# ChrisHekmanOtoy/opencl_render

Measured on AMD Instinct MI355X. Metric: Mrays/s (primary rays; each also traces its shadow/bounce rays) at ms/frame = ms_per_step, higher is better.
Workload: dtype f32

## Files before the change

include/raytrace_hip.h:

```cpp
#ifndef RAYTRACE_HIP_H
#define RAYTRACE_HIP_H

#include <stddef.h>
#include <stdint.h>
#include <time.h>

#ifdef __cplusplus
extern "C" {
#endif

#ifndef __OPENCL_CL_H
typedef int32_t  cl_int;
typedef uint32_t cl_uint;
typedef uint16_t cl_ushort;
typedef uint8_t  cl_uchar;
typedef int8_t   cl_char;
typedef float    cl_float;
typedef cl_uint  cl_bool;
typedef union { cl_float s[2]; } __attribute__((aligned(8)))  cl_float2;
typedef union { cl_uint  s[2]; } __attribute__((aligned(8)))  cl_uint2;
typedef union { cl_int   s[2]; } __attribute__((aligned(8)))  cl_int2;
typedef union { cl_float s[4]; } __attribute__((aligned(16))) cl_float4;
typedef union { cl_int   s[4]; } __attribute__((aligned(16))) cl_int4;
typedef union { cl_uchar s[4]; } __attribute__((aligned(4)))  cl_uchar4;
// ... 345 lines not shown
    char name[64];
    cl_float kd[3];
    cl_float ke[3]; cl_int hasKe;
    cl_float dissolve;
    cl_float reflect; cl_int hasReflect;
    char map[5][256];
} rtHipObjMaterial;
typedef struct rtHipObjData {
    cl_uint pointCount; cl_float3 *points;
    cl_uint polygonCount; cl_int *polygons; cl_float3 *cornerNormals; cl_float2 *cornerUv; cl_int *polygonMaterial;
    cl_uint materialCount; rtHipObjMaterial *materials;
} rtHipObjData;
int  rtHipObjRead(const char *path, rtHipObjData *out);
void rtHipObjFree(rtHipObjData *data);

int rtHipImageRead(const char *path, cl_uint *width, cl_uint *height, cl_uchar3 **pixels);

enum { RT_PROJ_SPHERICAL = 0, RT_PROJ_CYLINDRICAL = 1, RT_PROJ_FLAT = 2, RT_PROJ_CUBIC = 3, RT_PROJ_FRONTAL = 4, RT_PROJ_SPATIAL = 5,
       RT_PROJ_UVW = 6, RT_PROJ_SHRINKWRAP = 7, RT_PROJ_VOLUMESHADER = 10 };
int rtHipProjectUv(int projection, const cl_float point[3], const cl_float normal[3], cl_float offsetX, cl_float offsetY, cl_float lengthX,
                   cl_float lengthY, int tile, cl_float uv[2]);

void rtHipPlanesToRgb8(cl_uint width, cl_uint height, const cl_ushort *red, const cl_ushort *green, const cl_ushort *blue,
                       cl_uchar *rgb, int lowByteCompat);

int rtHipWriteBmp(const char *path, cl_uint width, cl_uint height, const cl_ushort *red, const cl_ushort *green, const cl_ushort *blue,
                  int lowByteCompat);

int rtHipWritePpm(const char *path, cl_uint width, cl_uint height, const cl_ushort *red, const cl_ushort *green, const cl_ushort *blue);

int rtHipWritePgm(const char *path, cl_uint width, cl_uint height, const cl_ushort *plane);
int rtHipWritePfm(const char *path, cl_uint width, cl_uint height, const cl_float *plane);
int rtHipWritePfmRgb(const char *path, cl_uint width, cl_uint height, const cl_float *rgb);

enum { RT_KAT_RANDF = 0, RT_KAT_SPHERE, RT_KAT_PMODF, RT_KAT_TRI, RT_KAT_PLINE, RT_KAT_BOX, RT_KAT_BIND, RT_KAT_POW, RT_KAT_QUOTIENT,
       RT_KAT_SPHERE_SPLIT, RT_KAT_ACCUM, RT_KAT_OPS };
int rtHipDeviceKat(int device, int op, cl_uint count, const void *in, cl_uint inStride, void *out, cl_uint outStride, const float *table);

enum { RT_SHADE_KAT_TEXEL = 0, RT_SHADE_KAT_NORMAL = 1 };
int rtHipTestShadeKat(const rtHipScene *scene, int op, cl_uint count, const void *in, void *out);

int rtHipTune(const char *key, double value);

int rtHipTestCachePointers(const void *out[6]);

uint64_t rtHipTestHashBytes(const void *bytes, uint64_t count);

int rtHipScenePathClass(const rtHipSceneDesc *desc);

int rtHipTestPathClass(const rtHipScene *scene);

int rtHipTestRoundLog(const rtHipScene *scene, cl_uint *rays, cl_uint n);

int rtHipTestShadeLog(const rtHipScene *scene, cl_uint *listed, cl_uint n);

enum { RT_BUILD_LOG_CAM_THREAD = 0, RT_BUILD_LOG_CAM_GROUP, RT_BUILD_LOG_CAM_ENTRIES, RT_BUILD_LOG_GRID_THREAD, RT_BUILD_LOG_GRID_GROUP,
       RT_BUILD_LOG_GRID_BATCHES, RT_BUILD_LOG_KEY_CAP_FIRST, RT_BUILD_LOG_KEY_CAP_FINAL, RT_BUILD_LOG_GREW, RT_BUILD_LOG_ATTEMPTS,
       RT_BUILD_LOG_PAIRS, RT_BUILD_LOG_FIELDS };
int rtHipTestBuildLog(uint64_t *out, cl_uint n);

enum { RT_SCENE_VIEW_HEADER = 0, RT_SCENE_VIEW_CAM_START, RT_SCENE_VIEW_CAM_END, RT_SCENE_VIEW_TRI_REC, RT_SCENE_VIEW_TRI_SHADE,
       RT_SCENE_VIEW_GRID_BITS, RT_SCENE_VIEW_BLOCK_SPARSE, RT_SCENE_VIEW_PAIR_REC, RT_SCENE_VIEW_CELL_LUT, RT_SCENE_VIEWS };
int rtHipTestSceneView(const rtHipScene *scene, int what, uint64_t firstElement, uint64_t count, void *out);

int rtHipTestSceneCameraList(const rtHipScene *scene, uint64_t first, uint64_t count, cl_uint *out);
int rtHipTestScenePointers(const rtHipScene *scene, const void *out[6]);
int rtHipTestSceneCameraLog(const rtHipScene *scene, uint64_t out[3]);
int rtHipTestSceneCameraTimes(const rtHipScene *scene, double out[2]);

int rtHipTestSceneGeometryLog(const rtHipScene *scene, uint64_t *out, cl_uint n);
int rtHipTestSceneGeometryTimes(const rtHipScene *scene, double ms[4]);

#ifdef __cplusplus
}
#endif
#endif
```

opencl_render_amd/csrc/rt_api.cpp:

```cpp
#include "rt_host.h"
#include "rt_build_shared.h"

#include <cmath>
#include <cstdarg>
#include <cstdio>
#include <cstdlib>
#include <unordered_map>
#include <chrono>

using namespace rthost;

extern "C" hipError_t rtk_launch_trace(const RtDevScene *scene, int counted, hipStream_t stream);
extern "C" hipError_t rtk_launch_prepare(uint32_t triangleCount, const void *vertex, const void *triIndex, const void *triMaterial,
                                         const void *triUv, const void *triNormal, float *triRec, float *triShade, hipStream_t stream);
extern "C" hipError_t rtk_launch_gather_pairs(uint32_t pairCount, const uint32_t *pairTri, const uint32_t *pairInfo, const float *triRec, float *pairRec, hipStream_t stream);
extern "C" hipError_t rtk_launch_detile(const void *tileBuf, const uint32_t *tileIds, uint32_t tileCount, uint32_t width,
                                        uint32_t height, uint32_t tilesX, void *planeR, void *planeG, void *planeB, int accumulate, hipStream_t stream);

extern "C" hipError_t rtp_validate(uint32_t T, uint32_t V, uint32_t M, const void *triIndex, const int *triMaterial, uint64_t camListSize,
                                   const uint32_t *camList, const uint32_t *gridStart, uint64_t gridListSize, const uint32_t *gridList, uint32_t *err,
                                   hipStream_t stream);
extern "C" hipError_t rtp_camera_ranges(uint32_t W, uint32_t H, uint32_t tilesX, const uint32_t *tileIds, uint32_t tileCount, const uint32_t *camStart,
                                        const uint32_t *camEnd, uint64_t camListSize, uint32_t *outStart, uint32_t *outEnd, uint32_t *err, hipStream_t stream);
extern "C" hipError_t rtp_dense_grid(const uint32_t *gridStart, const uint32_t *gridList, unsigned long long *words, uint32_t *sparse, uint32_t *pairOrder,
                                     uint32_t *pairCount, void *scratch, size_t *scratchBytes, hipStream_t stream);

extern "C" hipError_t rtc_scan_bytes(uint32_t n, size_t *bytes);
extern "C" hipError_t rtc_launch_count(const RtCamMoveArgs *args, hipStream_t stream);
extern "C" hipError_t rtc_launch_fill(const RtCamMoveArgs *args, hipStream_t stream);
extern "C" hipError_t rtw_launch_primary(const RtDevScene *scene, const RtWavefront *wf, hipStream_t stream);
extern "C" hipError_t rtw_launch_primary_passes(const RtDevScene *scene, const RtWavefront *wf, uint32_t *passBuf, hipStream_t stream);
extern "C" hipError_t rtw_launch_surface_passes(const RtDevScene *scene, const RtWavefront *wf, float *surfBuf, hipStream_t stream);
extern "C" hipError_t rtw_launch_logic(const RtDevScene *scene, const RtWavefront *wf, uint32_t round, uint32_t blocks, uint32_t slicesIn, const RtRoundMode *next, hipStream_t stream);
extern "C" hipError_t rtw_launch_answer(const RtDevScene *scene, const RtWavefront *wf, uint32_t round, uint32_t blocks, uint32_t slicesIn, const RtShadeList *list,
                                        uint32_t shadeFollows, hipStream_t stream);
extern "C" hipError_t rtw_launch_shade(const RtDevScene *scene, const RtWavefront *wf, uint32_t round, uint32_t blocks, uint32_t slicesIn, const RtRoundMode *next,
                                       const RtShadeList *list, hipStream_t stream);
extern "C" hipError_t rtw_launch_scatter(const RtWavefront *wf, uint32_t round, uint32_t blocks, const RtRoundMode *mode, hipStream_t stream);
extern "C" hipError_t rtw_launch_trace(const RtDevScene *scene, const RtWavefront *wf, uint32_t round, uint32_t blocks, const RtRoundMode *mode, hipStream_t stream);
extern "C" hipError_t rtw_launch_status(const RtWavefront *wf, uint32_t round, uint32_t *shadeCount, hipStream_t stream);
extern "C" hipError_t rtw_launch_accum(const RtDevScene *scene, const RtWavefront *wf, int first, hipStream_t stream);
extern "C" hipError_t rtw_launch_query(const RtDevScene *scene, const void *rays, const uint32_t *excluded, uint32_t count, void *hits,
                                       uint32_t fastQuotient, hipStream_t stream);
extern "C" hipError_t rtw_launch_ao(const RtDevScene *scene, const RtAoArgs *args, hipStream_t stream);
extern "C" hipError_t rtw_launch_motion_mark(const float *triRec, void *ref, uint32_t triangles, hipStream_t stream);
extern "C" hipError_t rtw_launch_motion(const RtDevScene *scene, const RtMotionArgs *args, hipStream_t stream);
extern "C" hipError_t rtw_launch_ao_finish(const RtDevScene *scene, const uint32_t *counter, uint32_t samplesTimesRays, float *out, uint32_t rowMajor,
                                           hipStream_t stream);
extern "C" hipError_t rtw_launch_bake_raster(const RtDevScene *scene, const RtBakeArgs *args, hipStream_t stream);
extern "C" hipError_t rtw_launch_bake_points(const RtDevScene *scene, const RtBakeArgs *args, hipStream_t stream);
extern "C" hipError_t rtw_launch_bake_ao(const RtDevScene *scene, const RtBakeArgs *args, hipStream_t stream);
extern "C" hipError_t rtw_launch_bake_finish(uint32_t texels, const uint32_t *win, const uint32_t *counter, uint32_t rays, float fill, float *out,
                                             uint32_t *tri, hipStream_t stream);
extern "C" hipError_t rtw_launch_bake_dilate(uint32_t W, uint32_t H, const float *src, float *dst, uint32_t last, hipStream_t stream);

namespace {
thread_local std::string g_error;
}

int rthost::fail(const char *fmt, ...)
{
    char buf[512];
    va_list ap;
    va_start(ap, fmt);
    vsnprintf(buf, sizeof buf, fmt, ap);
    va_end(ap);
    g_error = buf;
    return -1;
}

namespace {

Tuning g_tune;
std::mutex g_tuneMutex;
Tuning tuning() { std::lock_guard<std::mutex> lock(g_tuneMutex); return g_tune; }

// ... 75 lines not shown
    D.camStart = ts; D.camEnd = te;
    HIP_OK(hipStreamSynchronize(sc->stream));
    return 0;
}

int build_geometry(rtHipScene *sc, const rtHipSceneDesc *d)
{
    sc->release_part(PART_GEOMETRY);
    sc->curPart = PART_GEOMETRY;
    RtDevScene &D = sc->dev;
    D.triangleCount = d->triangleCount;
    if (d->triangleCount && (!d->triIndex || !d->triMaterial || !d->triUv || !d->triNormal)) return fail("null triangle array");
    if (d->vertexCount && !d->vertex) return fail("null vertex array");
    void *dv = nullptr, *di = nullptr, *dm = nullptr, *du = nullptr, *dn = nullptr;
    const uint64_t T = d->triangleCount, V = d->vertexCount;
    DevScratch scratch;
    HIP_OK(scratch.get(&dv, V * 16)); HIP_OK(scratch.get(&di, T * 16)); HIP_OK(scratch.get(&dm, T * 4));
    HIP_OK(scratch.get(&du, T * 24)); HIP_OK(scratch.get(&dn, T * 48));
    HIP_OK(sc->stager.copy(dv, d->vertex, V * 16));
    HIP_OK(sc->stager.copy(di, d->triIndex, T * 16));
    HIP_OK(sc->stager.copy(dm, d->triMaterial, T * 4));
    HIP_OK(sc->stager.copy(du, d->triUv, T * 24));
    HIP_OK(sc->stager.copy(dn, d->triNormal, T * 48));
    float *rec = nullptr, *shade = nullptr;
    if (sc->alloc<float>(T * 16, &rec) || sc->alloc<float>(T * 24, &shade)) return -1;
    HIP_OK(rtp_validate(d->triangleCount, d->vertexCount, d->materialCount, di, (const int *)dm, 0, nullptr, nullptr, 0, nullptr, sc->prepErr, sc->stream));
    HIP_OK(hipStreamSynchronize(sc->stream));
    if (sc->check_prep() != 0) return -1;
    HIP_OK(rtk_launch_prepare(d->triangleCount, dv, di, dm, du, dn, rec, shade, sc->stream));
    D.triRec = rec; D.triShade = shade;
    HIP_OK(hipStreamSynchronize(sc->stream));
    return 0;
}

void grid_tables(const float *planes, uint8_t *lut, uint32_t *tame)
{
    for (int w = 0; w < 3; ++w) {
        const float *pw = planes + w * (RT_GRID_DIV + 1);
        const float lo = pw[0], step = (pw[RT_GRID_DIV] - pw[0]) / 256.f;
        int c = 0;
        for (int i = 0; i < 256; ++i) {
            const float x = lo + ((float)i + 0.5f) * step;
            while (c < RT_GRID_DIV - 1 && pw[c + 1] < x) ++c;
            lut[w * 256 + i] = (uint8_t)c;
        }
    }
    *tame = 1u;
    for (int i = 0; i < 3 * (RT_GRID_DIV + 1); ++i) {
        const float m = std::fabs(planes[i]);
        if (!(m == 0.f || (m >= 0x1p-60f && m <= 0x1p39f))) *tame = 0u;
    }
}

int build_grid(rtHipScene *sc, const rtHipSceneDesc *d)
{
    sc->release_part(PART_GRID);
    sc->curPart = PART_GRID;
    RtDevScene &D = sc->dev;
    if (!d->boxMin) return fail("null sceneBoxMin");
    std::vector<float> planes(3 * (RT_GRID_DIV + 1));
    for (int w = 0; w < 3; ++w)
        for (int i = 0; i <= RT_GRID_DIV; ++i) planes[w * (RT_GRID_DIV + 1) + i] = d->boxMin[i].s[w];
    if (sc->upload(planes.data(), planes.size(), &D.boxMin, "boxMin")) return -1;
    std::vector<uint8_t> lut(3 * 256);
    grid_tables(planes.data(), lut.data(), &D.planesTame);
    if (sc->upload(lut.data(), lut.size(), &D.cellLut, "cellLut")) return -1;
    const uint64_t cells = (uint64_t)RT_GRID_DIV * RT_GRID_DIV * RT_GRID_DIV;
    if (!d->gridStart) return fail("null scenePixelTriangleListStart");
    const uint64_t listSize = sc->haveGridListSize ? sc->gridListSizeHint : d->gridStart[cells];
    if (listSize && !d->gridList) return fail("null scenePixelTriangleList");
    if (sc->upload(d->gridStart, cells + 1, &D.gridStart, "gridStart")) return -1;
    if (sc->upload(d->gridList, listSize, &D.gridList, "gridList")) return -1;
    HIP_OK(rtp_validate(D.triangleCount, 0, 0, nullptr, nullptr, 0, nullptr, D.gridStart, listSize, D.gridList, sc->prepErr, sc->stream));
    HIP_OK(hipStreamSynchronize(sc->stream));
    if (sc->check_prep() != 0) return -1;
    const size_t blocks = (size_t)(RT_GRID_DIV / 4) * (RT_GRID_DIV / 4) * (RT_GRID_DIV / 4);
    unsigned long long *words = nullptr;
    uint32_t *sparse = nullptr;
    const size_t sparseWords = (size_t)3 * ((63u << 16 | 63u << 8 | 63u) + 1u);
    if (listSize >= RT_PAIR_LIMIT) return fail("scenePixelTriangleList has 2^28 entries or more: pair indices would not fit the trace kernel's records");
    if (sc->alloc<unsigned long long>(blocks, &words) || sc->alloc<uint32_t>(sparseWords, &sparse)) return -1;
    HIP_OK(hipMemsetAsync(sparse, 0, sparseWords * 4, sc->stream));
    DevScratch scratch;
    uint32_t *pairOrder = nullptr, *pairCount = nullptr;
    void *tmp = nullptr;
    size_t tmpBytes = 0;
    HIP_OK(rtp_dense_grid(nullptr, nullptr, nullptr, nullptr, nullptr, nullptr, nullptr, &tmpBytes, sc->stream));
    HIP_OK(scratch.get((void **)&pairOrder, (size_t)listSize * 4)); HIP_OK(scratch.get((void **)&pairCount, (size_t)listSize * 4));
    HIP_OK(scratch.get(&tmp, tmpBytes));
    HIP_OK(rtp_dense_grid(D.gridStart, D.gridList, words, sparse, pairOrder, pairCount, tmp, &tmpBytes, sc->stream));
    float *pairRec = nullptr;
    if (sc->alloc<float>((uint64_t)listSize * 16, &pairRec)) return -1;
    HIP_OK(rtk_launch_gather_pairs((uint32_t)listSize, pairOrder, pairCount, D.triRec, pairRec, sc->stream));
    D.gridBits = words; D.gridBlockSparse = sparse; D.pairRec = pairRec;
    sc->gridListSize = listSize;
    D.cellCount = 0;
    HIP_OK(hipStreamSynchronize(sc->stream));
    return 0;
}

bool materials_admit_opaque_diffuse(const rtHipSceneDesc *d)
{
    for (uint32_t m = 0; m < d->materialCount; ++m)
        for (int c = 1; c < 5; ++c) {
            const uint32_t w = d->matSize[5 * m + c].s[0], h = d->matSize[5 * m + c].s[1];
            if (w == 0u) continue;
            if (w != 1u || h != 1u) return false;
            if (c == 3) continue;
            const cl_uchar *px = d->textures[d->matStart[5 * m + c]].s;
            if (px[0] | px[1] | px[2]) return false;
        }
    return true;
}
bool lights_admit_opaque_diffuse(const rtHipSceneDesc *d) { return d->lightCount <= 1u; }
void derive_path_class(rtHipScene *sc)
{
    sc->dev.pathClass = (sc->tune.logicClass && sc->classMaterials && sc->classLights) ? RT_PATH_CLASS_OPAQUE_DIFFUSE : RT_PATH_CLASS_GENERAL;
}

int build_materials(rtHipScene *sc, const rtHipSceneDesc *d)
{
    sc->release_part(PART_MATERIALS);
    sc->curPart = PART_MATERIALS;
    RtDevScene &D = sc->dev;
    D.materialCount = d->materialCount;
    D.texelCount = d->texturesSize ? d->texturesSize : 1;
    if (sc->upload((const uint32_t *)d->matSize, (uint64_t)d->materialCount * 10, &D.matSize, "materialImageSize")) return -1;
    if (sc->upload((const int32_t *)d->matStart, (uint64_t)d->materialCount * 5, &D.matStart, "materialImageStart")) return -1;
    if (sc->upload((const uint8_t *)d->textures, (uint64_t)d->texturesSize * 4, &D.textures, "textures")) return -1;
    for (uint32_t m = 0; m < d->materialCount * 5; ++m) {
        const uint64_t w = d->matSize[m].s[0], h = d->matSize[m].s[1];
        if (w && ((int64_t)d->matStart[m] < 0 || (uint64_t)d->matStart[m] + w * h > d->texturesSize))
            return fail("material channel %u: %llux%llu texels at %d exceed the %u-texel atlas", m, (unsigned long long)w, (unsigned long long)h, d->matStart[m], d->texturesSize);
    }
    {
        std::vector<uint32_t> rec((size_t)d->materialCount * 8, 0u);
        for (uint32_t m = 0; m < d->materialCount; ++m)
            for (int c = 0; c < 5; ++c) {
                const uint32_t w = d->matSize[5 * m + c].s[0], h = d->matSize[5 * m + c].s[1];
                uint32_t desc = 0u;
                if (w == 1u && h == 1u) {
                    const cl_uchar *px = d->textures[d->matStart[5 * m + c]].s;
                    desc = 0x80000000u | (uint32_t)px[0] | ((uint32_t)px[1] << 8) | ((uint32_t)px[2] << 16);
                } else if (w) desc = 0x40000000u;
                rec[8 * (size_t)m + c] = desc;
            }
        if (sc->upload(rec.data(), rec.size(), &D.matRec, "matRec")) return -1;
    }
    sc->classMaterials = materials_admit_opaque_diffuse(d);
    derive_path_class(sc);
// ... 102 lines not shown
        Wf.lookAhead = T.lookAhead ? 1u : 0u;
        Wf.deadShadow = T.deadShadow ? 1u : 0u;
        const uint64_t qcap = 2 * cap;
        const uint64_t extraCap = (uint64_t)extraFactor * cap;
        const uint64_t ecap = qcap + extraCap;
        if (ecap > 0xfffffff0ull) return fail("tile set too large for one batch");
        Wf.extraCap = (uint32_t)extraCap;
        Wf.sampleBase = 0; Wf.samplesInBatch = (uint32_t)sb;
        if (sc->alloc<unsigned long long>(cap, &Wf.rng) || sc->alloc<uint4>(cap, &Wf.meta) || sc->alloc<float4>(cap, &Wf.outc) ||
            sc->alloc<float4>(cap * RT_RING * 3, &Wf.ring) || sc->alloc<float4>(cap, &Wf.shP) || sc->alloc<float4>(cap, &Wf.shFace) ||
            sc->alloc<float4>(cap, &Wf.shAtt) || sc->alloc<float4>(multiLight ? cap : 1, &Wf.shN) ||
            sc->alloc<unsigned long long>(multiLight ? cap : 1, &Wf.rngL) || sc->alloc<unsigned long long>(cap, &Wf.laKey) ||
            sc->alloc<uint4>(ecap * 4, &Wf.ent[0]) || sc->alloc<uint4>(ecap * 4, &Wf.ent[1]) || sc->alloc<uint2>(cap, &Wf.pathOf[0]) ||
            sc->alloc<uint2>(cap, &Wf.pathOf[1]) || sc->alloc<unsigned long long>(qcap, &Wf.hitKey[0]) || sc->alloc<unsigned long long>(qcap, &Wf.hitKey[1]) ||
            sc->alloc<uint4>(cap, &Wf.res) || sc->alloc<float4>(gpix * sb, &Wf.sampleOut) ||
            sc->alloc<uint32_t>(ecap, &Wf.sortRank) || sc->alloc<uint16_t>(ecap, &Wf.sortTag) || sc->alloc<uint32_t>(ecap, &Wf.sortedIdx) ||
            sc->alloc<uint32_t>((uint64_t)3 * RT_WF_CTL_WORDS, &Wf.ctl) ||
            sc->alloc<uint4>(cap, &G.shade.list) || sc->alloc<uint32_t>((uint64_t)3 * RT_WF_SHARDS, &G.shade.count))
            return -1;
        HIP_OK(hipMemsetAsync(Wf.ctl, 0, sizeof(uint32_t) * 3 * RT_WF_CTL_WORDS, sc->stream));
        HIP_OK(hipMemsetAsync(G.shade.count, 0, sizeof(uint32_t) * 3 * RT_WF_SHARDS, sc->stream));
        HIP_OK(G.hostLog.make(sizeof(uint4) * RT_WF_ROUND_LOG, hipHostMallocMapped));
        memset(G.hostLog, 0, sizeof(uint4) * RT_WF_ROUND_LOG);
        HIP_OK(hipHostGetDevicePointer((void **)&Wf.roundLog, G.hostLog, 0));
        HIP_OK(G.hostCount.make(sizeof(uint32_t) * RT_WF_SHARDS, hipHostMallocDefault));
        HIP_OK(G.hostStatus.make(sizeof(uint32_t) * RT_WF_STATUS_WORDS, hipHostMallocMapped));
        memset(G.hostStatus, 0, sizeof(uint32_t) * RT_WF_STATUS_WORDS);
        HIP_OK(hipHostGetDevicePointer((void **)&Wf.hostStatus, G.hostStatus, 0));
        Wf.spinLimit = T.spinLimit ? T.spinLimit : 16384u;
        Wf.fastQuotient = T.fastQuotient ? 1u : 0u;
        G.queueBlocks = std::min<uint32_t>(cus * 16, (uint32_t)(qcap / 256));
        G.traceBlocks = (uint32_t)(ecap / 256);
        G.logicBlocks = std::min<uint32_t>(cus * 8, (uint32_t)((cap + 255) / 256));
        G.logicBlocks = std::max<uint32_t>(RT_WF_SHARDS / 4, (G.logicBlocks + RT_WF_SHARDS / 4 - 1) / (RT_WF_SHARDS / 4) * (RT_WF_SHARDS / 4));
    }
    HIP_OK(hipStreamSynchronize(sc->stream));
    sc->blocking = T.blocking != 0;
    return 0;
}

void refresh_views(rtHipScene *sc)
{
    const RtDevScene &D = sc->dev;
    for (auto &G : sc->groups) {
        G.dev = D;
        G.dev.tileIds = D.tileIds + G.slot0;
        G.dev.tileCount = G.slot1 - G.slot0;
        G.dev.camStart = D.camStart + (size_t)G.slot0 * RT_TILE_PIXELS;
        G.dev.camEnd = D.camEnd + (size_t)G.slot0 * RT_TILE_PIXELS;
        G.dev.tileBuf = D.tileBuf + (size_t)G.slot0 * 3 * RT_TILE_PIXELS;
    }
}

constexpr uint64_t GEO_PLANE_BYTES = 3 * (RT_GRID_DIV + 1) * 4, GEO_LUT_BYTES = 3 * 256, GEO_START_BYTES = ((uint64_t)RT_GRID_DIV * RT_GRID_DIV * RT_GRID_DIV + 1) * 4,
                   GEO_BITS_BYTES = (uint64_t)(RT_GRID_DIV / 4) * (RT_GRID_DIV / 4) * (RT_GRID_DIV / 4) * 8,
                   GEO_SPARSE_BYTES = (uint64_t)3 * ((63u << 16 | 63u << 8 | 63u) + 1u) * 4;

int clone_part(rtHipScene *dst, const rtHipScene *src, int part)
{
    dst->release_part(part);
    dst->curPart = part;
    std::vector<std::pair<const char *, char *>> moved;
    std::vector<void *> blocks = src->partAllocs[part];
    std::vector<uint64_t> sizes = src->partSizes[part];
    if (src->geo.live >= 0 && (part == PART_GEOMETRY || part == PART_GRID)) {
        const rtHipScene::GeoMove::Set &L = src->geo.set[src->geo.live];
        const uint64_t T = src->dev.triangleCount ? src->dev.triangleCount : 1, n = src->gridListSize ? src->gridListSize : 1;
        if (part == PART_GEOMETRY) { blocks = { L.triRec, L.triShade }; sizes = { T * 64, T * 96 }; }
        else {
            blocks = { L.boxMin, L.cellLut, L.gridStart, L.gridList, L.gridBits, L.sparse, L.pairRec };
            sizes = { GEO_PLANE_BYTES, GEO_LUT_BYTES, GEO_START_BYTES, n * 4, GEO_BITS_BYTES, GEO_SPARSE_BYTES, n * 64 };
        }
    }
    for (size_t i = 0; i < blocks.size(); ++i) {
        char *p = nullptr;
        const uint64_t n = sizes[i];
        if (dst->alloc<char>(n, &p)) return -1;
        HIP_OK(hipMemcpyPeerAsync(p, dst->device, blocks[i], src->device, n, dst->stream));
        moved.emplace_back((const char *)blocks[i], p);
    }
    auto at = [&](const void *old) -> const void * {
        for (auto &m : moved) if (m.first == (const char *)old) return m.second;
        return nullptr;
    };
    const RtDevScene &S = src->dev;
    RtDevScene &D = dst->dev;
#define RT_MOVE(field) D.field = (decltype(D.field))at(S.field)
    if (part == PART_GEOMETRY) { D.triangleCount = S.triangleCount; RT_MOVE(triRec); RT_MOVE(triShade); }
    if (part == PART_GRID) {
        D.planesTame = S.planesTame; D.cellCount = S.cellCount; dst->gridListSize = src->gridListSize;
        RT_MOVE(boxMin); RT_MOVE(cellLut); RT_MOVE(gridStart); RT_MOVE(gridList); RT_MOVE(gridBits); RT_MOVE(gridBlockSparse); RT_MOVE(pairRec);
    }
    if (part == PART_MATERIALS) {
        D.materialCount = S.materialCount; D.texelCount = S.texelCount; RT_MOVE(matSize); RT_MOVE(matStart); RT_MOVE(textures); RT_MOVE(matRec);
        dst->classMaterials = src->classMaterials;
        derive_path_class(dst);
    }
    if (part == PART_LIGHTS) {
        D.lightCount = S.lightCount;
        dst->classLights = src->classLights;
        derive_path_class(dst);
        RT_MOVE(lightType); RT_MOVE(lightPos); RT_MOVE(lightDir); RT_MOVE(lightCol); RT_MOVE(lightRadius); RT_MOVE(lightHalfAtt); RT_MOVE(lightSpread);
    }
#undef RT_MOVE
    HIP_OK(hipStreamSynchronize(dst->stream));
    return 0;
}

int scene_build(rtHipScene *sc, const rtHipSceneDesc *d, const cl_uint *tileIds, cl_uint tileCount, const rtHipScene *like, const Tuning &tune)
{
    if (!d) return fail("null scene description");
    if (d->width == 0 || d->height == 0) return fail("empty image %ux%u", d->width, d->height);
    if (d->sampleCount == 0) return fail("sampleCount must be >= 1");
    if (d->axesDiv != RT_GRID_DIV) return fail("axesDivCount %d unsupported (the reference builds %d, trianglelist.h:110)", d->axesDiv, RT_GRID_DIV);
    if ((uint64_t)d->width * d->height > 0xffffffffull) return fail("image too large");
    HIP_OK(hipSetDevice(sc->device));
    HIP_OK(sc->stream.make(hipStreamNonBlocking));
    sc->tune = tune;
    sc->pipeline = tune.pipeline == RT_HIP_PIPELINE_MEGAKERNEL ? RT_HIP_PIPELINE_MEGAKERNEL : RT_HIP_PIPELINE_WAVEFRONT;
    if (sc->stager.init(sc->stream, tune) != 0) return -1;
    const bool timing = tune.timing != 0;
    auto tLast = std::chrono::steady_clock::now();
    auto mark = [&](const char *what) {
        if (!timing) return;
        (void)hipStreamSynchronize(sc->stream);
        const auto now = std::chrono::steady_clock::now();
        fprintf(stderr, "libraytrace_hip: scene build: %-28s %8.1f ms\n", what, std::chrono::duration<double, std::milli>(now - tLast).count());
        tLast = now;
    };
    rtHipSceneDesc shadowed;
    std::vector<char> hostCopies[10];
    cl_uint gridEnd[1] = { 0 };
    if (d->arraysOnDevice) {
        shadowed = *d;
        auto fetch = [&](int slot, const void *&field, size_t bytes) -> int {
            if (!field || !bytes) return 0;
            hostCopies[slot].resize(bytes);
            HIP_OK(hipMemcpy(hostCopies[slot].data(), field, bytes, hipMemcpyDeviceToHost));
            field = hostCopies[slot].data();
            return 0;
        };
        const uint64_t cells = (uint64_t)RT_GRID_DIV * RT_GRID_DIV * RT_GRID_DIV;
        if (d->gridStart) { HIP_OK(hipMemcpy(gridEnd, d->gridStart + cells, 4, hipMemcpyDeviceToHost)); sc->gridListSizeHint = gridEnd[0]; sc->haveGridListSize = true; }
        if (fetch(0, (const void *&)shadowed.boxMin, (size_t)(RT_GRID_DIV + 1) * 16) || fetch(1, (const void *&)shadowed.matSize, (size_t)d->materialCount * 40) ||
            fetch(2, (const void *&)shadowed.matStart, (size_t)d->materialCount * 20) || fetch(3, (const void *&)shadowed.textures, (size_t)d->texturesSize * 4) ||
            fetch(4, (const void *&)shadowed.lightType, (size_t)d->lightCount * 4) || fetch(5, (const void *&)shadowed.lightPos, (size_t)d->lightCount * 16) ||
            fetch(6, (const void *&)shadowed.lightDir, (size_t)d->lightCount * 16) || fetch(7, (const void *&)shadowed.lightCol, (size_t)d->lightCount * 16) ||
            fetch(8, (const void *&)shadowed.lightRadius, (size_t)d->lightCount * 4) || fetch(9, (const void *&)shadowed.lightHalfAtt, (size_t)d->lightCount * 4))
            return -1;
        d = &shadowed;
    }
    if (build_fixed(sc, d, tileIds, tileCount) != 0) return -1;
    mark("tiles, outputs, bump tables");
    if (like) {
        for (int part : { PART_GEOMETRY, PART_GRID, PART_MATERIALS, PART_LIGHTS })
            if (clone_part(sc, like, part) != 0) return -1;
        mark("geometry, grid, materials, lights (copied from another instance)");
        if (build_camera(sc, d) != 0) return -1;
        mark("camera lists");
    } else {
        if (build_geometry(sc, d) != 0) return -1;
        mark("geometry");
        if (build_grid(sc, d) != 0) return -1;
        mark("grid + dense view");
        if (build_camera(sc, d) != 0) return -1;
        mark("camera lists");
        if (build_materials(sc, d) != 0) return -1;
        if (build_lights(sc, d) != 0) return -1;
        mark("materials + lights");
    }
    HIP_OK(rtp_validate(sc->dev.triangleCount, 0, 0, nullptr, nullptr, sc->camListSize, sc->dev.camList, nullptr, 0, nullptr, sc->prepErr, sc->stream));
    HIP_OK(hipStreamSynchronize(sc->stream));
    HIP_OK(sc->stager.drain());
    if (sc->check_prep() != 0) return -1;
    if (build_wavefront(sc, d->sampleCount) != 0) return -1;
    refresh_views(sc);
    mark("path state buffers");
    return 0;
}

RtRoundMode mode_for(const Tuning &T, uint32_t round, uint64_t rays, uint32_t slicesBefore)
{
    RtRoundMode m;
    m.ordered = (round <= 1u || rays >= T.appendRays) ? 1u : 0u;
    if (T.orderedFirst == 0u && rays < T.appendRays) m.ordered = 0u;
    m.segLen = rays >= T.segRays[0] ? T.segLen[0] : (rays >= T.segRays[1] ? T.segLen[1] : (rays >= T.segRays[2] ? T.segLen[2] : (rays >= T.segRays[3] ? T.segLen[3] : T.segLen[4])));
    if (m.segLen < 1u) m.segLen = 1u;
    uint32_t small = T.smallSlices;
    if (small < 1u || small > RT_WF_SHARDS || (small & (small - 1u))) small = 16u;
    m.slices = rays >= T.sliceRays ? (uint32_t)RT_WF_SHARDS : small;
    if (m.slices > slicesBefore) m.slices = slicesBefore;
    m.groupRays = (uint32_t)std::min<uint64_t>(64, std::max<uint64_t>(16, ((rays + 1099) / 1100 + 15) / 16 * 16));
    if (T.groupRays >= 1u && T.groupRays <= 128u) m.groupRays = T.groupRays;
    return m;
}

int render_wavefront(rtHipScene *sc, hipStream_t st, bool forceDiscovery)
{
    const Tuning &T = sc->tune;
    auto stage = [&](int which, hipStream_t on, auto &&launch) -> hipError_t {
        if (!sc->stageTiming) return launch();
        if (sc->stageEventsUsed == sc->stageEvents.size()) {
            rtHipScene::StageEvent e{};
            hipError_t er = e.a.make();
            if (er != hipSuccess) return er;
            er = e.b.make();
            if (er != hipSuccess) return er;
            sc->stageEvents.push_back(std::move(e));
        }
        rtHipScene::StageEvent &e = sc->stageEvents[sc->stageEventsUsed++];
        e.stage = which;
        hipError_t er = hipEventRecord(e.a, on);
        if (er != hipSuccess) return er;
        er = launch();
        if (er != hipSuccess) return er;
        return hipEventRecord(e.b, on);
    };
    const bool serial = sc->stageTiming || sc->groups.size() == 1;
    auto streamOf = [&](size_t g) { return (serial || g == 0) ? st : sc->groups[g].stream; };
    if (!serial) {
        HIP_OK(hipEventRecord(sc->forkEvent, st));
        for (size_t g = 1; g < sc->groups.size(); ++g) HIP_OK(hipStreamWaitEvent(sc->groups[g].stream, sc->forkEvent, 0));
    }
    const bool watchedFrame = forceDiscovery || sc->blocking || sc->planRounds == 0;
    bool planned = !watchedFrame;
    uint32_t planRounds = sc->planRounds;
    auto round_mode = [&](rtHipScene::Group &G, uint32_t r) -> RtRoundMode {
        if (G.modes.size() <= r) {
            const uint32_t before = G.modes.empty() ? (uint32_t)RT_WF_SHARDS : G.modes.back().slices;
            uint64_t rays = G.guessRays;
            if (planned) rays = r < RT_WF_ROUND_LOG ? G.plan[r].rays : 0;
            else G.guessRays = std::max<uint64_t>(G.guessRays / 4, 1);
            G.modes.resize(r + 1, mode_for(T, r, rays, before));
        }
        return G.modes[r];
    };
    auto trace_blocks = [&](rtHipScene::Group &G, uint32_t r, const RtRoundMode &m) -> uint32_t {
        const uint64_t worst = m.ordered ? G.traceBlocks : 2ull * G.wf.capacity / m.groupRays + 2ull * m.slices;
        if (!planned || r >= RT_WF_ROUND_LOG) return (uint32_t)std::min<uint64_t>(worst, 0x7fffffffu);
        if (T.planGridTiny) return 1;
        const uint64_t rays = G.plan[r].rays;
        const uint64_t extra = std::min<uint64_t>(G.wf.extraCap, G.plan[r].extraSegLen == m.segLen ? G.plan[r].extra : (m.segLen >= 4096u ? 0 : rays * 11));
        const uint64_t want = m.ordered ? ((rays + extra) * 11 / 10 + 255) / 256 + 8 : (rays * 11 / 10 + m.groupRays - 1) / m.groupRays + 2ull * m.slices + 8;
        return (uint32_t)std::max<uint64_t>(std::min<uint64_t>(want, worst), 1);
    };
    auto shade_blocks = [&](rtHipScene::Group &G, uint32_t r, const RtRoundMode &m) -> uint32_t {
        if (!planned || r >= RT_WF_ROUND_LOG) return G.logicBlocks;
        const uint64_t listed = T.planShadeSkip ? 0 : G.plan[r].shade;
        if (listed == 0) return 0;
        const uint64_t perSlice = (listed * 11 / 10 + m.slices - 1) / m.slices + 8;
        const uint64_t waves = (perSlice + 63) / 64 * m.slices, unit = RT_WF_SHARDS / 4;
        return (uint32_t)std::min<uint64_t>(G.logicBlocks, ((waves + 3) / 4 + unit - 1) / unit * unit);
    };
    uint64_t splitRounds = 0;
    auto issue_round = [&](rtHipScene::Group &G, hipStream_t on) -> int {
        const uint32_t r = G.rounds;
        const RtRoundMode mode = r > 0 ? round_mode(G, r) : RtRoundMode{ 0u, 4096u, 64u, (uint32_t)RT_WF_SHARDS };
        if (r > 0) {
            if (mode.ordered) HIP_OK(stage(4, on, [&] { return rtw_launch_scatter(&G.wf, r, G.queueBlocks, &mode, on); }));
            HIP_OK(stage(2, on, [&] { return rtw_launch_trace(&G.dev, &G.wf, r, trace_blocks(G, r, mode), &mode, on); }));
        }
        const RtRoundMode next = round_mode(G, r + 1);
        if (r > 0 && T.logicSplit && G.wf.lookAhead && G.dev.pathClass == RT_PATH_CLASS_OPAQUE_DIFFUSE) {
            const uint32_t shadeBlocks = shade_blocks(G, r, mode);
            ++splitRounds;
            HIP_OK(stage(1, on, [&] { return rtw_launch_answer(&G.dev, &G.wf, r, G.logicBlocks, mode.slices, &G.shade, shadeBlocks ? 1u : 0u, on); }));
            if (shadeBlocks) HIP_OK(stage(1, on, [&] { return rtw_launch_shade(&G.dev, &G.wf, r, shadeBlocks, mode.slices, &next, &G.shade, on); }));
        } else
            HIP_OK(stage(1, on, [&] { return rtw_launch_logic(&G.dev, &G.wf, r, G.logicBlocks, mode.slices, &next, on); }));
        ++G.rounds;
        return 0;
    };
    auto issue_chunk = [&](rtHipScene::Group &G, hipStream_t on) -> int {
        for (uint32_t k = 0; k < 3 && G.rounds < RT_WF_MAX_ROUNDS; ++k)
            if (issue_round(G, on) != 0) return -1;
        HIP_OK(hipMemcpyAsync(G.hostCount, G.wf.ctl + (G.rounds % 3) * RT_WF_CTL_WORDS + RT_WF_CTL_COUNTS, sizeof(uint32_t) * RT_WF_SHARDS, hipMemcpyDeviceToHost, on));
        return 0;
    };
    auto device_error = [&](rtHipScene::Group &G) -> int {
        if (const uint32_t err = G.hostStatus[RT_WF_STATUS_ERROR]) {
            G.hostStatus[RT_WF_STATUS_ERROR] = 0u;
            return fail("wavefront pipeline: device error 0x%x%s -- the frame is invalid", err,
                        (err & RT_WF_ERR_SPIN) ? " (wf_trace_kernel's walk guard tripped: rays were abandoned)" : "");
        }
        return 0;
    };
    auto launch_surface = [&](rtHipScene::Group &G, hipStream_t on) {
        return rtw_launch_surface_passes(&G.dev, &G.wf, sc->surfBuf + (size_t)G.slot0 * RT_SURF_WORDS * RT_TILE_PIXELS, on);
    };
    uint64_t rounds = 0;
    bool anyPlannedBatch = false;
    const uint32_t sampleCount = sc->dev.sampleCount;
    for (uint32_t base = 0; base < sampleCount; base += sc->samplesPerBatch) {
        for (size_t g = 0; g < sc->groups.size(); ++g) {
            rtHipScene::Group &G = sc->groups[g];
            const hipStream_t on = streamOf(g);
            G.wf.sampleBase = base;
            G.wf.samplesInBatch = std::min<uint32_t>(sc->samplesPerBatch, sampleCount - base);
            G.rounds = 0;
            G.modes.clear();
            G.guessRays = (uint64_t)(G.slot1 - G.slot0) * RT_TILE_PIXELS * G.wf.samplesInBatch;
            if (!G.ctlClean) {
                HIP_OK(hipMemsetAsync(G.wf.ctl, 0, sizeof(uint32_t) * (size_t)3 * RT_WF_CTL_WORDS, on));
                HIP_OK(hipMemsetAsync(G.shade.count, 0, sizeof(uint32_t) * (size_t)3 * RT_WF_SHARDS, on));
            }
            G.ctlClean = false;
            if (!planned) memset(G.hostLog, 0, sizeof(uint4) * RT_WF_ROUND_LOG);
            if (sc->passBuf) {
                uint32_t *pass = sc->passBuf + (size_t)G.slot0 * RT_PASS_WORDS * RT_TILE_PIXELS;
                HIP_OK(stage(0, on, [&] {
                    if (base == 0 && sampleCount > 1) {
                        const hipError_t er = hipMemset2DAsync(pass + RT_PASS_HITS * RT_TILE_PIXELS, (size_t)RT_PASS_WORDS * RT_TILE_PIXELS * 4, 0,
                                                               (size_t)RT_TILE_PIXELS * 4, G.slot1 - G.slot0, on);
// ... 1033 lines not shown
    GEO_MEM(geo_set_fit(sc, target, false, 0, 0, true, &allocated), "the spare set of records and grid arrays");
    GEO_MEM(geo_fit(sc, G.material, T * 4, true, &allocated), "the build scratch");
    if (allocated) GEO_HIP(hipMemsetAsync(G.material, 0xff, (size_t)G.material.size, st));

    const void *dVertex = up->vertex, *dIndex = up->triIndex, *dNormal = up->triNormal;
    if (!up->arraysOnDevice) {
        GEO_MEM(geo_fit(sc, G.vertexBuf, V * 16, false, &allocated), "the vertices");
        GEO_HIP(sc->stager.copy(G.vertexBuf, up->vertex, V * 16));
        dVertex = G.vertexBuf;
        GEO_MEM(geo_fit(sc, G.normalBuf, T * 48, true, &allocated), "the corner normals");
        if (up->triNormal) {
            GEO_HIP(sc->stager.copy(G.normalBuf, up->triNormal, T * 48));
            dNormal = G.normalBuf;
        }
    }
    GEO_MEM(geo_fit(sc, G.index[0], T * 16, true, &allocated) && geo_fit(sc, G.index[1], T * 16, true, &allocated), "the index arrays");
    if (up->triIndex) {
        GEO_HIP(sc->stager.copy(G.index[spareIndex], up->triIndex, T * 16));
        dIndex = G.index[spareIndex];
    } else dIndex = G.index[G.retained];
    GEO_HIP(sc->stager.drain());
    GEO_HIP(hipEventRecord(G.ev[0], st));

    GEO_HIP(rtp_validate((uint32_t)T, (uint32_t)V, 0x7fffffffu, dIndex, G.material, 0, nullptr, nullptr, 0, nullptr, sc->prepErr, st));
    GEO_HIP(hipStreamSynchronize(st));
    if (sc->check_prep() != 0) return -5;

    GEO_HIP(rtg_launch_records((uint32_t)T, dVertex, dIndex, dNormal, sc->dev.triShade, N.triRec, N.triShade, st));
    GEO_HIP(hipEventRecord(G.ev[1], st));

    uint64_t pairs = 0, glog[RT_BUILD_LOG_FIELDS] = {};
    G.space.allocated = 0;
    const uint64_t spaceBefore = G.space.bytes;
    const int grc = rt_grid_core_fill(&G.space, (uint32_t)V, (uint32_t)T, dVertex, dIndex, tune.buildKeyCap, listLimit, st, &pairs, glog);
    sc->bytes += G.space.bytes - spaceBefore;
    allocated = allocated || G.space.allocated;
    if (grc == -3) { fail("%s: the grid holds %llu pairs, more than the limit of %llu", who, (unsigned long long)glog[RT_BUILD_LOG_PAIRS], (unsigned long long)listLimit); return -3; }
    if (grc == -7) { fail("%s: a single triangle's fill outgrew its workgroup queue, or the second fill overflowed", who); return -7; }
    if (grc == -4) { fail("%s: no device memory for the grid build", who); return -4; }
    if (grc) { fail("%s: the grid build failed on the device", who); return -2; }
    if (pairs >= RT_PAIR_LIMIT) { fail("%s: the grid holds 2^28 pairs or more: pair indices would not fit the trace kernel's records", who); return -3; }
    GEO_MEM(geo_set_fit(sc, target, true, pairs * 4, pairs * 64, false, &allocated), "the grid list and pair records");
    GEO_MEM(geo_fit(sc, G.pairOrder, pairs * 4, false, &allocated) && geo_fit(sc, G.pairInfo, pairs * 4, false, &allocated), "the pair order");
    if (rt_grid_core_lists(&G.space, pairs, N.gridStart, N.gridList, st) != 0) { fail("%s: sorting the grid's pairs failed on the device", who); return -2; }
    float bm[4 * (RT_GRID_DIV + 1)];
    GEO_HIP(hipMemcpyAsync(bm, G.space.bm, sizeof bm, hipMemcpyDeviceToHost, st));
    GEO_HIP(hipStreamSynchronize(st));
    float planes[3 * (RT_GRID_DIV + 1)];
    uint8_t lut[3 * 256];
    uint32_t tame = 0;
    for (int w = 0; w < 3; ++w)
        for (int i = 0; i <= RT_GRID_DIV; ++i) planes[w * (RT_GRID_DIV + 1) + i] = bm[4 * i + w];
    grid_tables(planes, lut, &tame);
    GEO_HIP(hipMemcpyAsync(N.boxMin, planes, sizeof planes, hipMemcpyHostToDevice, st));
    GEO_HIP(hipMemcpyAsync(N.cellLut, lut, sizeof lut, hipMemcpyHostToDevice, st));
    GEO_HIP(hipEventRecord(G.ev[2], st));

    size_t denseBytes = 0;
    GEO_HIP(rtp_dense_grid(nullptr, nullptr, nullptr, nullptr, nullptr, nullptr, nullptr, &denseBytes, st));
    GEO_MEM(geo_fit(sc, G.denseTmp, denseBytes, true, &allocated), "the dense view's scratch");
    denseBytes = (size_t)G.denseTmp.size;
    GEO_HIP(hipMemsetAsync(N.sparse, 0, GEO_SPARSE_BYTES, st));
    GEO_HIP(rtp_dense_grid(N.gridStart, N.gridList, N.gridBits, N.sparse, G.pairOrder, G.pairInfo, G.denseTmp, &denseBytes, st));
    GEO_HIP(rtk_launch_gather_pairs((uint32_t)pairs, G.pairOrder, G.pairInfo, N.triRec, N.pairRec, st));
    GEO_HIP(hipEventRecord(G.ev[3], st));

    rtHipCamera cam;
    (void)rtHipSceneGetCamera(sc, &cam);
    int camTarget = 0;
    RtCamMoveCtl ctl{};
    float camMs[2] = { 0.f, 0.f };
    if (const int rc = cam_move_build(sc, &cam, N.triRec, N.triShade, listLimit, who, &camTarget, &ctl, camMs)) return rc;
    GEO_HIP(hipEventRecord(G.ev[4], st));
    GEO_HIP(hipStreamSynchronize(st));
    float ms[4] = {};
    for (int i = 0; i < 4; ++i) GEO_HIP(hipEventElapsedTime(&ms[i], G.ev[i], G.ev[i + 1]));
#undef GEO_HIP
#undef GEO_MEM

    RtDevScene &D = sc->dev;
    D.triRec = N.triRec; D.triShade = N.triShade;
    D.boxMin = N.boxMin; D.cellLut = N.cellLut; D.planesTame = tame;
    D.gridStart = N.gridStart; D.gridList = N.gridList; D.gridBits = N.gridBits; D.gridBlockSparse = N.sparse; D.pairRec = N.pairRec;
    sc->gridListSize = pairs;
    G.live = target;
    if (up->triIndex) G.retained = spareIndex;
    sc->cam.args.triRec = N.triRec; sc->cam.args.triShade = N.triShade;
    cam_move_commit(sc, &cam, camTarget, ctl);
    sc->release_part(PART_GEOMETRY);
    sc->release_part(PART_GRID);
    (void)geo_set_fit(sc, target ^ 1, true, N.gridList.size, N.pairRec.size, true, &allocated);
    allocated = allocated || camMade || camCapBefore[0] != sc->cam.list[0].size || camCapBefore[1] != sc->cam.list[1].size;
    G.log[0] = glog[RT_BUILD_LOG_GRID_THREAD]; G.log[1] = glog[RT_BUILD_LOG_GRID_GROUP]; G.log[2] = glog[RT_BUILD_LOG_ATTEMPTS];
    G.log[3] = pairs; G.log[4] = ctl.total; G.log[5] = allocated ? 1 : 0;
    for (int i = 0; i < 4; ++i) G.ms[i] = ms[i];
    return 0;
}

int rtHipTestSceneGeometryLog(const rtHipScene *sc, uint64_t *out, cl_uint n)
{
    if (!sc || (n && !out)) return fail("rtHipTestSceneGeometryLog: null argument");
    for (cl_uint i = 0; i < n; ++i) out[i] = i < 6 ? sc->geo.log[i] : 0;
    return 6;
}

int rtHipTestSceneGeometryTimes(const rtHipScene *sc, double ms[4])
{
    if (!sc || !ms) return fail("rtHipTestSceneGeometryTimes: null argument");
    for (int i = 0; i < 4; ++i) ms[i] = sc->geo.ms[i];
    return 0;
}

int rtHipKernelTime(rtHipScene *sc, double *avgMs, uint64_t *launches)
{
    if (!sc || !avgMs || !launches) return fail("null argument");
    HIP_OK(hipSetDevice(sc->device));
    double total = 0.0;
    for (size_t i = 0; i < sc->eventsUsed; ++i) {
        HIP_OK(hipEventSynchronize(sc->events[i].second));
        float ms = 0.f;
        HIP_OK(hipEventElapsedTime(&ms, sc->events[i].first, sc->events[i].second));
        total += ms;
    }
    *launches = sc->eventsUsed;
    *avgMs = sc->eventsUsed ? total / (double)sc->eventsUsed : 0.0;
    sc->eventsUsed = 0;
    return 0;
}


static std::atomic<cl_bool> g_tableReady{ CL_FALSE };
static std::atomic<int> g_deviceCount{ 0 };
static char g_deviceName[256][256];
static std::mutex g_tableMutex;

// ... 105 lines not shown
            chunks[i].h = chunks[i].p ? hash_chunk(chunks[i].p, chunks[i].n) : mix64(chunks[i].n + 0x51ull);
    };
    std::vector<std::thread> pool;
    for (unsigned t = 1; t < threads; ++t) pool.emplace_back(work);
    work();
    for (auto &t : pool) t.join();
    for (int g = 0; g < 5; ++g) out[g] = 0x12345678u + g;
    for (const Chunk &c : chunks) out[c.group] = mix64(out[c.group] * 0x100000001b3ull ^ c.h);
}

struct SceneCache {
    std::vector<rtHipScene *> scenes;
    std::vector<std::vector<cl_uint>> tiles;
    int first = 0, count = 0, devices = 0;
    Tuning tune;
    uint32_t width = 0, height = 0, sampleCount = 0;
    uint64_t hash[5] = { 0 };
    bool valid = false;
    Dev<uint16_t> planes, gather;
    Dev<uint32_t> gatherIds;
    uint64_t bytes = 0;
    size_t gatherTiles = 0;
    void clear()
    {
        for (rtHipScene *s : scenes) rtHipSceneDestroy(s);
        scenes.clear(); tiles.clear();
        if (valid || planes || gather || gatherIds) {
            if (devices > 0) (void)hipSetDevice(first % devices);
            planes.drop(bytes); gather.drop(bytes); gatherIds.drop(bytes);
        }
        gatherTiles = 0;
        valid = false;
    }
};
SceneCache &g_cache = *new SceneCache();
std::mutex g_cacheMutex;

}

extern "C" {

int rtHipTune(const char *key, double value)
{
    if (!key) return fail("rtHipTune: null key");
    std::lock_guard<std::mutex> lock(g_tuneMutex);
    Tuning &T = g_tune;
    const std::string k = key;
    if (k == "reset") { T = Tuning(); return 0; }
    struct Key { const char *name; uint32_t *f32; uint64_t *f64 = nullptr; double most = 4294967295.0; } table[] = {
        { "stage_mb", &T.stageMb }, { "extra_factor", &T.extraFactor }, { "groups", &T.groups }, { "lookahead", &T.lookAhead },
        { "seg0", &T.segLen[0] }, { "seg1", &T.segLen[1] }, { "seg2", &T.segLen[2] }, { "seg3", &T.segLen[3] }, { "seg4", &T.segLen[4] },
        { "seg_rays0", &T.segRays[0] }, { "seg_rays1", &T.segRays[1] }, { "seg_rays2", &T.segRays[2] }, { "seg_rays3", &T.segRays[3] },
        { "fast_quotient", &T.fastQuotient }, { "spin_limit", &T.spinLimit }, { "append_rays", &T.appendRays }, { "ordered_first", &T.orderedFirst }, { "slice_rays", &T.sliceRays },
        { "small_slices", &T.smallSlices }, { "group_rays", &T.groupRays }, { "blocking", &T.blocking }, { "plan_rounds", &T.planRounds }, { "plan_grid_tiny", &T.planGridTiny }, { "plan_shade_skip", &T.planShadeSkip },
        { "pipeline", &T.pipeline }, { "timing", &T.timing }, { "virtual_devices", &T.virtualDevices }, { "cache", &T.cache }, { "batch_plan", &T.batchPlan },
        { "logic_class", &T.logicClass }, { "dead_shadow", &T.deadShadow }, { "logic_split", &T.logicSplit }, { "query_rays", &T.queryRays, nullptr, 1u << 26 },
        { "ao_samples", &T.aoSamples, nullptr, 1u << 22 }, { "bake_texels", &T.bakeTexels, nullptr, 1u << 24 },
        { "state_mb", nullptr, &T.stateMb, HUGE_VAL }, { "build_key_cap", nullptr, &T.buildKeyCap, 1e18 }, { "build_list_limit", nullptr, &T.buildListLimit },
    };
    for (const Key &e : table) {
        if (k != e.name) continue;
        const double v = value < 0 ? 0 : std::min(value, e.most);
        if (e.f64) *e.f64 = (uint64_t)v; else *e.f32 = (uint32_t)v;
        return 0;
    }
    return fail("rtHipTune: unknown key '%s'", key);
}

int rtHipTestCachePointers(const void *out[6])
{
    if (!out) return -1;
    std::lock_guard<std::mutex> lock(g_cacheMutex);
    if (!g_cache.valid || g_cache.scenes.empty() || !g_cache.scenes[0]) return -2;
    const RtDevScene &D = g_cache.scenes[0]->dev;
    out[0] = D.triRec; out[1] = D.triShade; out[2] = D.pairRec; out[3] = D.matRec; out[4] = D.textures; out[5] = D.camList;
    return 0;
}

int rtHipTestPathClass(const rtHipScene *scene)
{
    if (!scene) return -1;
    return (int)scene->dev.pathClass;
}

int rt_shade_kat_run(const RtDevScene *scene, int op, uint32_t count, const void *in, void *out);

int rtHipTestShadeKat(const rtHipScene *scene, int op, uint32_t count, const void *in, void *out)
{
    if (!scene || (count && (!in || !out))) return -1;
    const RtDevScene &D = scene->dev;
    for (uint32_t i = 0; i < count; ++i) {
        if (op == RT_SHADE_KAT_TEXEL) {
            const int32_t *item = reinterpret_cast<const int32_t *>(in) + 10 * (size_t)i;
            if (D.texelCount == 0u || item[0] < 0 || (uint32_t)item[0] >= D.materialCount || item[1] < 0 || item[1] >= 5) return -1;
        } else if (op == RT_SHADE_KAT_NORMAL) {
            if (reinterpret_cast<const uint32_t *>(in)[12 * (size_t)i] >= D.triangleCount) return -1;
        } else return -1;
    }
    if (op == RT_SHADE_KAT_NORMAL && count && D.texelCount == 0u && D.materialCount) return -1;
    if (hipSetDevice(scene->device) != hipSuccess || hipStreamSynchronize(scene->stream) != hipSuccess) return -3;
    return rt_shade_kat_run(&D, op, count, in, out);
}

int rtHipTestRoundLog(const rtHipScene *scene, uint32_t *rays, uint32_t n)
{
    if (!scene || (n && !rays)) return -1;
    const uint32_t rounds = (uint32_t)std::min<uint64_t>(scene->roundsLast, RT_WF_ROUND_LOG);
    for (uint32_t r = 0; r < n; ++r) {
        uint64_t sum = 0;
        if (r < rounds)
            for (const auto &G : scene->groups) sum += G.hostLog[r].x;
        rays[r] = (uint32_t)std::min<uint64_t>(sum, 0xffffffffu);
    }
    return (int)scene->roundsLast;
}

int rtHipTestShadeLog(const rtHipScene *scene, uint32_t *listed, uint32_t n)
{
    if (!scene || (n && !listed)) return -1;
    const uint32_t rounds = (uint32_t)std::min<uint64_t>(scene->roundsLast, RT_WF_ROUND_LOG);
    for (uint32_t r = 0; r < n; ++r) {
        uint64_t sum = 0;
        if (r < rounds)
            for (const auto &G : scene->groups) sum += G.hostLog[r].w;
        listed[r] = (uint32_t)std::min<uint64_t>(sum, 0xffffffffu);
    }
    return (int)std::min<uint64_t>(scene->splitRoundsLast, 0x7fffffffu);
}

int rtHipTestSceneView(const rtHipScene *scene, int what, uint64_t firstElement, uint64_t count, void *out)
{
    if (!scene) return fail("rtHipTestSceneView: null scene");
    const RtDevScene &D = scene->dev;
    const uint32_t header[5] = { D.planesTame, D.tileCount, D.tilesX, D.triangleCount, (uint32_t)scene->gridListSize };
    const uint64_t tilePixels = (uint64_t)D.tileCount * RT_TILE_PIXELS, blocks = (uint64_t)(RT_GRID_DIV / 4) * (RT_GRID_DIV / 4) * (RT_GRID_DIV / 4);
    struct View { const void *ptr; uint64_t elements, elementBytes; bool host; } v;
    switch (what) {
    case RT_SCENE_VIEW_HEADER: v = { header, 5, 4, true }; break;
    case RT_SCENE_VIEW_CAM_START: v = { D.camStart, tilePixels, 4, false }; break;
    case RT_SCENE_VIEW_CAM_END: v = { D.camEnd, tilePixels, 4, false }; break;
    case RT_SCENE_VIEW_TRI_REC: v = { D.triRec, D.triangleCount, 64, false }; break;
    case RT_SCENE_VIEW_TRI_SHADE: v = { D.triShade, D.triangleCount, 96, false }; break;
    case RT_SCENE_VIEW_GRID_BITS: v = { D.gridBits, blocks, 8, false }; break;
    case RT_SCENE_VIEW_BLOCK_SPARSE: v = { D.gridBlockSparse, (uint64_t)3 * ((63u << 16 | 63u << 8 | 63u) + 1u), 4, false }; break;
    case RT_SCENE_VIEW_PAIR_REC: v = { D.pairRec, scene->gridListSize, 64, false }; break;
    case RT_SCENE_VIEW_CELL_LUT: v = { D.cellLut, 3 * 256, 1, false }; break;
    default: return fail("rtHipTestSceneView: unknown array %d", what);
    }
    if (v.elements > 0x7fffffffull) return fail("rtHipTestSceneView: array %d has %llu elements", what, (unsigned long long)v.elements);
    if (!out) return (int)v.elements;
    if (firstElement > v.elements || count > v.elements - firstElement)
        return fail("rtHipTestSceneView: elements %llu + %llu reach past the %llu of array %d", (unsigned long long)firstElement,
                    (unsigned long long)count, (unsigned long long)v.elements, what);
    if (!count) return 0;
    if (v.host) { memcpy(out, (const char *)v.ptr + firstElement * v.elementBytes, count * v.elementBytes); return 0; }
    if (!v.ptr) return fail("rtHipTestSceneView: the scene does not hold array %d", what);
    HIP_OK(hipSetDevice(scene->device));
    HIP_OK(hipStreamSynchronize(scene->stream));
    HIP_OK(hipMemcpy(out, (const char *)v.ptr + firstElement * v.elementBytes, count * v.elementBytes, hipMemcpyDeviceToHost));
    return 0;
}

int rtHipScenePathClass(const rtHipSceneDesc *desc)
{
    if (!desc) return fail("rtHipScenePathClass: null scene description");
    if (desc->arraysOnDevice) return fail("rtHipScenePathClass: the description's arrays are device memory");
    if (desc->materialCount && (!desc->matSize || !desc->matStart || !desc->textures)) return fail("rtHipScenePathClass: null material array");
    for (uint32_t i = 0; i < desc->materialCount * 5; ++i)
        if (desc->matSize[i].s[0] == 1u && desc->matSize[i].s[1] == 1u && ((int64_t)desc->matStart[i] < 0 || (uint64_t)desc->matStart[i] >= desc->texturesSize))
            return fail("rtHipScenePathClass: material channel %u starts outside the atlas", i);
    return (materials_admit_opaque_diffuse(desc) && lights_admit_opaque_diffuse(desc)) ? RT_PATH_CLASS_OPAQUE_DIFFUSE : RT_PATH_CLASS_GENERAL;
}

uint64_t rtHipTestHashBytes(const void *bytes, uint64_t count) { return hash_chunk((const unsigned char *)bytes, (size_t)count); }

void rtHipCacheClear(void)
{
    std::lock_guard<std::mutex> lock(g_cacheMutex);
    const std::string keep = g_error;
    g_cache.clear();
    g_error = keep;
}

cl_bool RaytraceAll(cl_uint computationType, cl_uint2 cameraImageDimension, cl_float3 cameraEye, cl_float3 cameraEyeToTopLeftVector,
                    cl_float3 cameraLeftToRightPixelSizeVector, cl_float3 cameraTopToBottomPixelSizeVector, cl_float cameraPixelSizeInv,
                    cl_uint *cameraPixelTriangleListStart, cl_uint *cameraPixelTriangleListEnd, cl_uint *cameraPixelTriangleList,
                    ptrdiff_t cameraPixelTriangleListSize, cl_uint sampleCount, cl_uint vertexCount, cl_float3 *vertex,
                    cl_uint triangleCount, cl_int3 *triangleVertexIndex, cl_int *triangleMaterialId, cl_float2 *triangleUv,
                    cl_float3 *triangleNormal, cl_int axesDivCount, cl_float3 *sceneBoxMin, cl_uint *scenePixelTriangleListStart,
                    cl_uint *scenePixelTriangleList, cl_uint materialCount, cl_uint2 *materialImageSize, cl_int *materialImageStart,
                    cl_uint texturesSize, cl_uchar3 *textures, cl_uint lightCount, cl_int *lightType, cl_float3 *lightPosition,
                    cl_float3 *lightDirection, cl_float3 *lightColour, cl_float *lightRadius, cl_float *lightHalfAttenuationDistance,
                    cl_ushort *outputRed, cl_ushort *outputGreen, cl_ushort *outputBlue)
{
    g_error.clear();
    auto refuse = [&](const char *why) -> cl_bool {
        fprintf(stderr, "libraytrace_hip: %s\n", why);
        return CL_FALSE;
    };
// ... 220 lines not shown
```

opencl_render_amd/csrc/rt_host.h:

```cpp
#pragma once
#include "raytrace_hip.h"
#include "rt_device.h"
#include "rt_camera_move.h"
#include "rt_geometry_move.h"
#include "rt_owned.h"

#include <hip/hip_runtime_api.h>

#include <algorithm>
#include <atomic>
#include <cstring>
#include <mutex>
#include <string>
#include <thread>
#include <vector>

#define RT_SURF_BUF_BITS (RT_HIP_PASS_NORMAL | RT_HIP_PASS_ALBEDO)

namespace rthost {

#define RT_INTERNAL __attribute__((visibility("hidden")))

RT_INTERNAL int fail(const char *fmt, ...);

#define HIP_OK(expr)                                                                                   \
    do {                                                                                               \
        hipError_t e_ = (expr);                                                                        \
        if (e_ != hipSuccess) return rthost::fail("%s failed: %s", #expr, hipGetErrorString(e_));      \
    } while (0)

struct Tuning {
    uint32_t stageMb = 32;
    uint32_t extraFactor = 6;
    uint64_t stateMb = 0;
    uint32_t groups = 1;
    uint32_t lookAhead = 1;
    uint32_t segLen[5] = { 4096u, 384u, 96u, 64u, 16u };
    uint32_t segRays[4] = { 700000u, 300000u, 100000u, 30000u };
    uint32_t fastQuotient = 1;
    uint32_t spinLimit = 16384;
    uint32_t appendRays = 300000;
    uint32_t orderedFirst = 1;
    uint32_t sliceRays = 0;
    uint32_t smallSlices = 16;
    uint32_t groupRays = 0;
    uint32_t blocking = 0;
    uint32_t planRounds = 0;
    uint32_t planGridTiny = 0;
    uint32_t planShadeSkip = 0;
    uint32_t pipeline = RT_HIP_PIPELINE_WAVEFRONT;
    uint32_t timing = 0;
    uint32_t virtualDevices = 0;
    uint32_t cache = 1;
    uint32_t batchPlan = 1;
    uint32_t logicClass = 1;
    uint32_t deadShadow = 1;
    uint32_t logicSplit = 1;
    uint64_t buildKeyCap = 0;
    uint64_t buildListLimit = 0xffffffffull;
    uint32_t queryRays = 1u << 20;
    uint32_t aoSamples = 1u << 20;
    uint32_t bakeTexels = 1u << 20;
};

struct DevScratch {
    std::vector<void *> blocks;
    ~DevScratch() { for (void *p : blocks) (void)hipFree(p); }
    hipError_t get(void **out, size_t bytes)
    {
        const hipError_t e = hipMalloc(out, bytes ? bytes : 1);
        if (e == hipSuccess) blocks.push_back(*out);
        return e;
    }
};

struct Stager {
    hipStream_t stream = nullptr;
    char *buf[2] = { nullptr, nullptr };
    hipEvent_t done[2] = { nullptr, nullptr };
    bool used[2] = { false, false };
    size_t size = 0;
    int next = 0;
    struct Pool {
        std::mutex lock;
        std::vector<std::pair<char *, size_t>> idle;
        char *take(size_t bytes)
        {
            {
                std::lock_guard<std::mutex> g(lock);
                for (size_t i = 0; i < idle.size(); ++i)
                    if (idle[i].second == bytes) { char *p = idle[i].first; idle.erase(idle.begin() + i); return p; }
            }
            char *p = nullptr;
            if (hipHostMalloc((void **)&p, bytes, hipHostMallocPortable) != hipSuccess) { (void)hipGetLastError(); return nullptr; }
            return p;
        }
        void give(char *p, size_t bytes)
        {
            std::lock_guard<std::mutex> g(lock);
            if (idle.size() < 8) idle.emplace_back(p, bytes);
            else (void)hipHostFree(p);
        }
    };
    static Pool &pool() { static Pool *p = new Pool(); return *p; }
    int init(hipStream_t st, const Tuning &T)
    {
        stream = st;
        size = (size_t)std::min<uint32_t>(std::max<uint32_t>(T.stageMb, 1u), 4096u) << 20;
        for (int i = 0; i < 2; ++i) HIP_OK(hipEventCreateWithFlags(&done[i], hipEventDisableTiming));
// ... 20 lines not shown
    {
        if (bytes && on_device(src)) return hipMemcpyAsync(dst, src, bytes, hipMemcpyDeviceToDevice, stream);
        for (size_t off = 0; off < bytes;) {
            const size_t n = std::min(size, bytes - off);
            const int i = next;
            next ^= 1;
            if (used[i]) { const hipError_t e = hipEventSynchronize(done[i]); if (e != hipSuccess) return e; }
            if (!buf[i] && !(buf[i] = pool().take(size))) return hipErrorOutOfMemory;
            fill(buf[i], (const char *)src + off, n);
            hipError_t e = hipMemcpyAsync((char *)dst + off, buf[i], n, hipMemcpyHostToDevice, stream);
            if (e != hipSuccess) return e;
            e = hipEventRecord(done[i], stream);
            if (e != hipSuccess) return e;
            used[i] = true;
            off += n;
        }
        return hipSuccess;
    }
    hipError_t drain()
    {
        for (int i = 0; i < 2; ++i) {
            if (used[i]) { const hipError_t e = hipEventSynchronize(done[i]); if (e != hipSuccess) return e; used[i] = false; }
            if (buf[i]) { pool().give(buf[i], size); buf[i] = nullptr; }
        }
        return hipSuccess;
    }
    void destroy()
    {
        for (int i = 0; i < 2; ++i) {
            if (done[i]) { if (used[i]) (void)hipEventSynchronize(done[i]); (void)hipEventDestroy(done[i]); done[i] = nullptr; }
            if (buf[i]) { pool().give(buf[i], size); buf[i] = nullptr; }
        }
    }
};

}

enum { PART_FIXED = 0, PART_CAMERA, PART_GEOMETRY, PART_GRID, PART_MATERIALS, PART_LIGHTS, PART_WAVEFRONT, PART_COUNT };

struct rtHipScene {
    int device = -1;
    rthost::Stream stream;
    RtDevScene dev{};
    std::vector<void *> partAllocs[PART_COUNT];
    std::vector<uint64_t> partSizes[PART_COUNT];
    uint64_t partBytes[PART_COUNT] = { 0 };
    int curPart = PART_FIXED;
    rthost::Stager stager;
    uint32_t *prepErr = nullptr;
    uint64_t camListSize = 0;
    uint64_t gridListSize = 0;
    uint32_t gridListSizeHint = 0;
    bool haveGridListSize = false;
    bool wfMultiLight = false;
    bool classMaterials = false, classLights = false;
    uint64_t bytes = 0;
    std::vector<cl_uint> tileIds;
    uint32_t width = 0, height = 0, tilesX = 0;
    std::vector<std::pair<rthost::Event, rthost::Event>> events;
    size_t eventsUsed = 0;
    int pipeline = RT_HIP_PIPELINE_WAVEFRONT;
    struct Group {
        RtDevScene dev{};
        RtWavefront wf{};
        RtShadeList shade{};
        rthost::Stream stream;
        rthost::Event done;
        uint32_t logicBlocks = 1, traceBlocks = 1, queueBlocks = 1;
        rthost::Pinned<uint32_t> hostCount;
        rthost::Pinned<uint32_t> hostStatus;
        bool ctlClean = false;
        uint32_t rounds = 0;
        uint32_t slot0 = 0, slot1 = 0;
        uint32_t roundsNeeded = 0;
        struct RoundPlan { uint32_t rays = 0, extra = 0, extraSegLen = 0, shade = 0; };
        rthost::Pinned<uint4> hostLog;
        RoundPlan plan[RT_WF_ROUND_LOG], planNext[RT_WF_ROUND_LOG];
        std::vector<RtRoundMode> modes;
        uint64_t guessRays = 0;
    };
    std::vector<Group> groups;
    rthost::Event forkEvent;
    uint32_t samplesPerBatch = 1;
    uint32_t planRounds = 0;
    uint64_t splitRoundsLast = 0;
    bool blocking = false;
    rthost::Tuning tune;
    bool unverified = false;
    hipStream_t lastStream = nullptr;
    rtHipSampleWindow window{}, lastWindow{};
    std::atomic<float> *progress = nullptr;
    float progressBase = 0.f, progressSpan = 0.f;
    struct StageEvent { int stage; rthost::Event a, b; };
    std::vector<StageEvent> stageEvents;
    size_t stageEventsUsed = 0;
    bool stageTiming = false;
    uint64_t roundsLast = 0;
    uint32_t passMask = 0;
    rthost::Dev<uint32_t> passBuf;
    rthost::Dev<float> surfBuf;
    uint32_t queryRays = 0;
    rthost::Dev<> queryDev;
    char *queryHost = nullptr;
    rthost::Dev<> denoiseBuf;
    rthost::Event denoiseEv[4];
    float denoiseMs[3] = {};
    rthost::Dev<> aoBuf;
    uint32_t aoChunk = 0;
    rthost::Event aoDone;
    rthost::Dev<> bakeBuf;
    uint64_t bakeTexels = 0;
    uint32_t bakeChunk = 0;
    rthost::Event bakeDone;
    struct Motion {
        bool have = false;
        rtHipCamera cam{};
        uint32_t triangles = 0;
        rthost::Dev<float4> ref;
        rthost::Dev<> stage;
        rthost::Event marked, done;
    } motion;
    struct Temporal {
        rthost::Dev<> buf, momentsBuf;
        int cur = 0;
        bool valid = false, momentsValid = false;
        rthost::Event ev[5];
        float ms[4] = {};
    } temporal;
    struct CamMove {
        rthost::Dev<> scratch;
        rthost::Dev<uint32_t> start[2], end[2], list[2];
        int live = -1;
        RtCamMoveArgs args{};
        rthost::Event ev[4];
        uint64_t log[3] = {};
        double ms[2] = {};
    } cam;
    struct GeoMove {
        struct Set {
            rthost::Dev<float> triRec, triShade, boxMin, pairRec;
            rthost::Dev<uint8_t> cellLut;
            rthost::Dev<uint32_t> gridStart, gridList, sparse;
            rthost::Dev<unsigned long long> gridBits;
        } set[2];
        int live = -1;
        RtGridSpace space{};
        rthost::Dev<> vertexBuf, normalBuf, index[2], denseTmp;
        rthost::Dev<int> material;
        rthost::Dev<uint32_t> pairOrder, pairInfo;
        int retained = -1;
// ... 90 lines not shown
```

opencl_render_amd/csrc/rt_scene_prep.hip:

```cpp
#include <hip/hip_runtime.h>
#include <hipcub/hipcub.hpp>

#include "rt_device.h"

namespace {

constexpr uint32_t BLOCKS = (RT_GRID_DIV / 4) * (RT_GRID_DIV / 4) * (RT_GRID_DIV / 4);

__global__ __launch_bounds__(256) void rtp_check_triangles(uint32_t T, uint32_t V, uint32_t M, const int4 *__restrict__ triIndex,
                                                           const int *__restrict__ triMaterial, uint32_t *err)
{
    const uint32_t t = blockIdx.x * 256 + threadIdx.x;
    if (t >= T) return;
    const int4 vi = triIndex[t];
    uint32_t bad = 0;
    if ((uint32_t)vi.x >= V || (uint32_t)vi.y >= V || (uint32_t)vi.z >= V) bad |= RT_PREP_ERR_TRI_INDEX;
    if (triMaterial[t] >= (int)M) bad |= RT_PREP_ERR_TRI_MATERIAL;
    if (bad) atomicOr(err, bad);
}

__global__ __launch_bounds__(256) void rtp_check_list(uint64_t n, const uint32_t *__restrict__ list, uint32_t T, uint32_t bit, uint32_t *err)
{
    const uint64_t i = (uint64_t)blockIdx.x * 256 + threadIdx.x;
    if (i < n && list[i] >= T) atomicOr(err, bit);
}

__global__ __launch_bounds__(256) void rtp_check_grid_start(const uint32_t *__restrict__ gridStart, uint32_t *err)
{
    const uint32_t c = blockIdx.x * 256 + threadIdx.x;
    if (gridStart[c] > gridStart[c + 1]) atomicOr(err, RT_PREP_ERR_GRID_MONOTONE);
}

__global__ __launch_bounds__(256) void rtp_camera_tile_major(uint32_t W, uint32_t H, uint32_t tilesX, const uint32_t *__restrict__ tileIds, uint32_t tileCount,
                                                             const uint32_t *__restrict__ camStart, const uint32_t *__restrict__ camEnd, uint64_t camListSize,
                                                             uint32_t *__restrict__ outStart, uint32_t *__restrict__ outEnd, uint32_t *err)
{
    const uint32_t i = blockIdx.x * 256 + threadIdx.x;
    if (i >= tileCount * RT_TILE_PIXELS) return;
    const uint32_t slot = i / RT_TILE_PIXELS, in = i % RT_TILE_PIXELS;
    const uint32_t tile = tileIds[slot];
    const uint32_t gx = (tile % tilesX) * RT_TILE + in % RT_TILE, gy = (tile / tilesX) * RT_TILE + in / RT_TILE;
    uint32_t a = 0, b = 0;
    if (gx < W && gy < H) {
        const uint64_t p = (uint64_t)gy * W + gx;
        a = camStart[p]; b = camEnd[p];
        if (b < a) b = a;
        if ((uint64_t)b > camListSize) { atomicOr(err, RT_PREP_ERR_CAM_RANGE); a = b = 0; }
    }
    outStart[i] = a; outEnd[i] = b;
}

__global__ __launch_bounds__(256) void rtp_block_words(const uint32_t *__restrict__ gridStart, unsigned long long *__restrict__ words,
                                                       uint32_t *__restrict__ blockCells, uint32_t *__restrict__ blockRest)
{
    const uint32_t b = blockIdx.x * 256 + threadIdx.x;
    const uint32_t bx = b & 63u, by = (b >> 6) & 63u, bz = b >> 12;
    unsigned long long w = 0;
    uint32_t cells = 0, rest = 0;
    for (uint32_t z = 0; z < 4; ++z)
        for (uint32_t y = 0; y < 4; ++y) {
            const uint32_t row = (bx * 4) + RT_GRID_DIV * (by * 4 + y) + RT_GRID_DIV * RT_GRID_DIV * (bz * 4 + z);
            uint32_t s[5];
#pragma unroll
            for (int x = 0; x < 5; ++x) s[x] = gridStart[row + x];
#pragma unroll
            for (uint32_t x = 0; x < 4; ++x) {
                const uint32_t n = s[x + 1] - s[x];
                if (n) { w |= 1ull << (x | (y << 2) | (z << 4)); ++cells; rest += n - 1; }
            }
        }
    words[b] = w; blockCells[b] = cells; blockRest[b] = rest;
}

__global__ __launch_bounds__(256) void rtp_block_emit(const uint32_t *__restrict__ gridStart, const uint32_t *__restrict__ gridList,
                                                      const unsigned long long *__restrict__ words, const uint32_t *__restrict__ rank,
                                                      const uint32_t *__restrict__ restBase, const uint32_t *__restrict__ blockCells,
                                                      uint32_t *__restrict__ sparse, uint32_t *__restrict__ pairOrder, uint32_t *__restrict__ pairCount)
{
    const uint32_t b = blockIdx.x * 256 + threadIdx.x;
    const uint32_t bx = b & 63u, by = (b >> 6) & 63u, bz = b >> 12;
    unsigned long long w = words[b];
    const uint32_t first = rank[b];
    const size_t at = (size_t)(bx | (by << 8) | (bz << 16)) * 3;
    sparse[at + 0] = (uint32_t)w; sparse[at + 1] = (uint32_t)(w >> 32); sparse[at + 2] = first;
    const uint32_t cellTotal = rank[BLOCKS - 1] + blockCells[BLOCKS - 1];
    uint32_t dense = first, restAt = cellTotal + restBase[b];
    while (w) {
        const int bit = __ffsll((long long)w) - 1;
        w &= w - 1;
        const uint32_t cell = (bx * 4 + (bit & 3)) + RT_GRID_DIV * (by * 4 + ((bit >> 2) & 3)) + RT_GRID_DIV * RT_GRID_DIV * (bz * 4 + (bit >> 4));
        const uint32_t s = gridStart[cell], n = gridStart[cell + 1] - s;
        pairOrder[dense] = gridList[s];
        pairCount[dense] = (n < RT_PAIR_MANY ? n : RT_PAIR_MANY) | (restAt << 4);
        for (uint32_t i = 1; i < n; ++i) { pairOrder[restAt] = gridList[s + i]; pairCount[restAt] = (i == 1u) ? n : 0u; ++restAt; }
        ++dense;
    }
}

}

extern "C" hipError_t rtp_validate(uint32_t T, uint32_t V, uint32_t M, const void *triIndex, const int *triMaterial, uint64_t camListSize,
                                   const uint32_t *camList, const uint32_t *gridStart, uint64_t gridListSize, const uint32_t *gridList, uint32_t *err,
                                   hipStream_t stream)
{
    if (T && triIndex) hipLaunchKernelGGL(rtp_check_triangles, dim3((T + 255) / 256), dim3(256), 0, stream, T, V, M, (const int4 *)triIndex, triMaterial, err);
    if (camListSize) hipLaunchKernelGGL(rtp_check_list, dim3((uint32_t)((camListSize + 255) / 256)), dim3(256), 0, stream, camListSize, camList, T, RT_PREP_ERR_CAM_ENTRY, err);
    if (gridListSize) hipLaunchKernelGGL(rtp_check_list, dim3((uint32_t)((gridListSize + 255) / 256)), dim3(256), 0, stream, gridListSize, gridList, T, RT_PREP_ERR_GRID_ENTRY, err);
    if (gridStart) hipLaunchKernelGGL(rtp_check_grid_start, dim3((RT_GRID_DIV * RT_GRID_DIV * RT_GRID_DIV) / 256), dim3(256), 0, stream, gridStart, err);
    return hipGetLastError();
}

extern "C" hipError_t rtp_camera_ranges(uint32_t W, uint32_t H, uint32_t tilesX, const uint32_t *tileIds, uint32_t tileCount, const uint32_t *camStart,
                                        const uint32_t *camEnd, uint64_t camListSize, uint32_t *outStart, uint32_t *outEnd, uint32_t *err, hipStream_t stream)
{
    const uint32_t n = tileCount * RT_TILE_PIXELS;
    if (n) hipLaunchKernelGGL(rtp_camera_tile_major, dim3((n + 255) / 256), dim3(256), 0, stream, W, H, tilesX, tileIds, tileCount, camStart, camEnd,
                              camListSize, outStart, outEnd, err);
    return hipGetLastError();
}

extern "C" hipError_t rtp_dense_grid(const uint32_t *gridStart, const uint32_t *gridList, unsigned long long *words, uint32_t *sparse, uint32_t *pairOrder,
                                     uint32_t *pairCount, void *scratch, size_t *scratchBytes, hipStream_t stream)
{
    size_t scanBytes = 0;
    hipError_t e = hipcub::DeviceScan::ExclusiveSum(nullptr, scanBytes, (const uint32_t *)nullptr, (uint32_t *)nullptr, (int)BLOCKS, stream);
    if (e != hipSuccess) return e;
    const size_t need = (size_t)4 * BLOCKS * sizeof(uint32_t) + scanBytes;
    if (!scratch) { *scratchBytes = need; return hipSuccess; }
    if (*scratchBytes < need) return hipErrorInvalidValue;
    uint32_t *blockCells = (uint32_t *)scratch, *blockRest = blockCells + BLOCKS, *rank = blockRest + BLOCKS, *restBase = rank + BLOCKS;
    void *scanTmp = restBase + BLOCKS;
    hipLaunchKernelGGL(rtp_block_words, dim3(BLOCKS / 256), dim3(256), 0, stream, gridStart, words, blockCells, blockRest);
    e = hipcub::DeviceScan::ExclusiveSum(scanTmp, scanBytes, blockCells, rank, (int)BLOCKS, stream);
    if (e != hipSuccess) return e;
    e = hipcub::DeviceScan::ExclusiveSum(scanTmp, scanBytes, blockRest, restBase, (int)BLOCKS, stream);
    if (e != hipSuccess) return e;
    hipLaunchKernelGGL(rtp_block_emit, dim3(BLOCKS / 256), dim3(256), 0, stream, gridStart, gridList, words, rank, restBase, blockCells, sparse, pairOrder,
                       pairCount);
    return hipGetLastError();
}
```

opencl_render_amd/csrc/rt_wavefront.hip:

```cpp
#include "rt_devfuncs.h"

namespace {

enum { WS_RAY = 0, WS_SHADOW = 1 };

__device__ __forceinline__ float4 pack4(V3 v, float w) { return make_float4(v.x, v.y, v.z, w); }
__device__ __forceinline__ V3 xyz(float4 v) { return mk(v.x, v.y, v.z); }

__device__ __forceinline__ void store_single_sample(const RtDevScene &S, uint32_t localPixel, V3 c)
{
    const uint32_t slot = localPixel / RT_TILE_PIXELS, inTile = localPixel % RT_TILE_PIXELS;
    uint16_t *planes = S.tileBuf + (size_t)slot * 3 * RT_TILE_PIXELS + inTile;
    uint32_t samples = S.sampleDivisor;
    asm volatile("" : "+s"(samples));
    const float scale = (float)(0xFFFF) / (float)samples;
    planes[0] = (uint16_t)sat_add_u16(0, c.x, scale);
    planes[RT_TILE_PIXELS] = (uint16_t)sat_add_u16(0, c.y, scale);
    planes[2 * RT_TILE_PIXELS] = (uint16_t)sat_add_u16(0, c.z, scale);
}

__device__ __forceinline__ uint32_t wave_append(uint32_t *counter, bool want)
{
    const unsigned long long mask = __ballot(want);
    if (mask == 0) return 0;
    const uint32_t lane = __lane_id();
    const int leader = __ffsll((long long)mask) - 1;
    uint32_t base = 0;
    if ((int)lane == leader) base = atomicAdd(counter, (uint32_t)__popcll(mask));
    base = __shfl(base, leader, 64);
    return base + (uint32_t)__popcll(mask & ((1ull << lane) - 1ull));
}

__device__ __forceinline__ void wave_append2(uint32_t *counterA, bool wantA, uint32_t *counterB, bool wantB, uint32_t &posA, uint32_t &posB)
{
    const unsigned long long maskA = __ballot(wantA), maskB = __ballot(wantB);
    const uint32_t lane = __lane_id();
    uint32_t base = 0;
    const uint32_t n = (lane == 0u) ? (uint32_t)__popcll(maskA) : (uint32_t)__popcll(maskB);
    if (lane < 2u && n != 0u) base = atomicAdd(lane == 0u ? counterA : counterB, n);
    const unsigned long long below = (1ull << lane) - 1ull;
    posA = (uint32_t)__shfl((int)base, 0, 64) + (uint32_t)__popcll(maskA & below);
    posB = (uint32_t)__shfl((int)base, 1, 64) + (uint32_t)__popcll(maskB & below);
}

__device__ __forceinline__ bool tri_rec_test_flat(const float4 r0, const float4 r1, const float4 r2, const float4 r3, V3 o, V3 d, float tmin,
                                                  float tmax, float &t, float &l1, float &l2)
{
    const V3 a = mk(r0.x, r0.y, r0.z), ab = mk(r0.w, r1.x, r1.y), ac = mk(r1.z, r1.w, r2.x), n = mk(r2.y, r2.z, r2.w);
    const V3 ao = sub3(o, a);
    t = -dot3(n, ao) / dot3(n, d);
    const V3 ap = sub3(along(o, t, d), a);
    const float ap_ab = dot3(ap, ab);
    const float ap_ac = dot3(ap, ac);
// ... 205 lines not shown
}

#ifndef RT_WF_MAXSEG
#define RT_WF_MAXSEG 12
#endif
struct DdaState { uint32_t cell; float dx, dy, dz; };

__device__ __forceinline__ uint32_t axis_state_at(const float *planes, uint32_t c0, float oa, float da, float tau, float &head,
                                                  const uint8_t *lut = nullptr, float lutScale = 0.f)
{
    const bool pos = (0.f <= da);
    const int limit = pos ? (int)(RT_GRID_DIV - 1 - c0) : (int)c0;
    const float p = oa + tau * da;
    int g = 0;
    bool search = true;
    if (lut) {
        const int i = min(255, max(0, (int)((p - planes[0]) * lutScale)));
        const int a = lut[max(i - 1, 0)], b = lut[min(i + 1, 255)];
        g = lut[i];
        search = b - a > 4;
    }
    if (search) {
        g = 0;
#pragma unroll
        for (int div = RT_GRID_DIV / 2; div >= 1; div /= 2)
            if (planes[g + div] < p) g += div;
    }
    int m = pos ? g - (int)c0 : (int)c0 - g;
    m = m < 0 ? 0 : (m > limit ? limit : m);
    while (m >= 1 && !((planes[pos ? (int)c0 + m : (int)c0 - m + 1] - oa) / da <= tau)) --m;
    float next = (planes[pos ? (int)c0 + m + 1 : (int)c0 - m] - oa) / da;
    while (m < limit && next <= tau) {
        ++m;
        next = (planes[pos ? (int)c0 + m + 1 : (int)c0 - m] - oa) / da;
    }
    head = next;
    return pos ? c0 + (uint32_t)m : c0 - (uint32_t)m;
}

__device__ __forceinline__ uint32_t cell_of(const float *planes, V3 p)
{
    int cx = 0, cy = 0, cz = 0;
#pragma unroll
    for (int div = RT_GRID_DIV / 2; div >= 1; div /= 2) {
        if (planes[cx + div] < p.x) cx += div;
        if (planes[(RT_GRID_DIV + 1) + cy + div] < p.y) cy += div;
        if (planes[2 * (RT_GRID_DIV + 1) + cz + div] < p.z) cz += div;
    }
    return (uint32_t)cx | ((uint32_t)cy << 8) | ((uint32_t)cz << 16);
}

struct EntryPlan { DdaState start; uint32_t endCell, visits; float te; };

__device__ __forceinline__ EntryPlan plan_ray(const float *planes, V3 o, V3 d, float tmin, float tmax, bool haveStart = false, uint32_t startCell = 0u,
                                              const uint8_t *lut = nullptr, const float *lutScale = nullptr)
{
    EntryPlan p;
    const V3 lo = mk(planes[0], planes[RT_GRID_DIV + 1], planes[2 * (RT_GRID_DIV + 1)]);
    const V3 hi = mk(planes[RT_GRID_DIV], planes[2 * RT_GRID_DIV + 1], planes[3 * RT_GRID_DIV + 2]);
    V3 from = along(o, tmin, d);
    bind_in_cube(from, d, lo, hi);
    p.start.cell = startCell;
    if (!haveStart) p.start.cell = cell_of(planes, from);
    p.te = RT_INF;
    V3 to;
    if (tmax < RT_INF) {
        to = along(o, tmax, d);
        bind_in_cube(to, d, lo, hi);
    } else {
        if (d.x != 0.f) { const float t = (((0.f <= d.x) ? hi.x : lo.x) - o.x) / d.x; if (t < p.te) p.te = t; }
        if (d.y != 0.f) { const float t = (((0.f <= d.y) ? hi.y : lo.y) - o.y) / d.y; if (t < p.te) p.te = t; }
        if (d.z != 0.f) { const float t = (((0.f <= d.z) ? hi.z : lo.z) - o.z) / d.z; if (t < p.te) p.te = t; }
        to = (p.te < RT_INF) ? along(o, p.te, d) : from;
    }
    uint32_t last;
    if (lut && !(tmax < RT_INF)) {
        const float fx = (to.x - lo.x) * lutScale[0], fy = (to.y - lo.y) * lutScale[1], fz = (to.z - lo.z) * lutScale[2];
        const int ix = min(255, max(0, (int)fx)), iy = min(255, max(0, (int)fy)), iz = min(255, max(0, (int)fz));
        last = (uint32_t)lut[ix] | ((uint32_t)lut[256 + iy] << 8) | ((uint32_t)lut[512 + iz] << 16);
    } else last = cell_of(planes, to);
    p.endCell = (tmax < RT_INF) ? last : 0xffffffffu;
    const int cx = (int)(p.start.cell & 255u), cy = (int)((p.start.cell >> 8) & 255u), cz = (int)(p.start.cell >> 16);
    p.start.dx = (planes[cx + ((0 <= d.x) ? 1 : 0)] - o.x) / d.x;
    p.start.dy = (planes[(RT_GRID_DIV + 1) + cy + ((0 <= d.y) ? 1 : 0)] - o.y) / d.y;
    p.start.dz = (planes[2 * (RT_GRID_DIV + 1) + cz + ((0 <= d.z) ? 1 : 0)] - o.z) / d.z;
    p.visits = (uint32_t)(abs((int)(last & 255u) - cx) + abs((int)((last >> 8) & 255u) - cy) + abs((int)(last >> 16) - cz)) + 1u;
    return p;
}

__device__ __forceinline__ uint32_t segments_of(const EntryPlan &p, V3 d, float tmax, uint32_t segLen)
{
    const float ta = fminf(p.start.dx, fminf(p.start.dy, p.start.dz));
    const bool plain = !(tmax < RT_INF) && d.x != 0.f && d.y != 0.f && d.z != 0.f && p.te < RT_INF && -RT_INF < ta && ta < p.te &&
                       p.start.dx == p.start.dx && p.start.dy == p.start.dy && p.start.dz == p.start.dz && p.start.dx < RT_INF &&
                       p.start.dy < RT_INF && p.start.dz < RT_INF;
    if (!plain || p.visits <= segLen + segLen / 4) return 1u;
    const uint32_t n = (p.visits + segLen - 1) / segLen;
    return n > RT_WF_MAXSEG ? (uint32_t)RT_WF_MAXSEG : n;
}

__device__ __forceinline__ bool cut_at(float ta, float te, uint32_t k, uint32_t n, float &tau)
{
    tau = ta + (te - ta) * ((float)k / (float)n);
    return ta <= tau && tau < te;
}

#ifndef RT_WF_LOGIC_WAVES
#define RT_WF_LOGIC_WAVES 3
#endif
#ifndef RT_WF_LOGIC_WAVES_FIRST
#define RT_WF_LOGIC_WAVES_FIRST 3
#endif
#ifndef RT_WF_LOGIC_WAVES_FIRST_ORDERED
#define RT_WF_LOGIC_WAVES_FIRST_ORDERED 3
#endif
#ifndef RT_WF_LOGIC_WAVES_LEAN_FIRST
#define RT_WF_LOGIC_WAVES_LEAN_FIRST 4
#endif
#ifndef RT_WF_LOGIC_WAVES_LEAN
#define RT_WF_LOGIC_WAVES_LEAN 4
#endif
#define RT_WF_LIGHTS_LDS 64
#ifdef RT_DIAG_LOGIC
#define DG(i) dg[i] = diag_stamp()
#else
#define DG(i)
#endif
__device__ __forceinline__ void class_light_accum(V3 &face, float ndl, bool front, float lmax, float4 lc, V3 atten)
{
    const float mag = __builtin_fabsf(ndl);
    const float x = lmax / lc.w;
    const float e = mag * half_falloff(x);
    if ((0.f <= ndl) == front) {
        face.x += (1.f - face.x) * atten.x * e * lc.x;
        face.y += (1.f - face.y) * atten.y * e * lc.y;
        face.z += (1.f - face.z) * atten.z * e * lc.z;
    }
}
__device__ __forceinline__ void class_shade_end(V3 &out, V3 P, V3 face)
{
    out.x += P.x * face.x;
    out.y += P.y * face.y;
    out.z += P.z * face.z;
}

__device__ __forceinline__ void log_round_rays(const RtWavefront &W, const uint32_t *ctlIn, uint32_t round, uint32_t lane, uint32_t wave)
{
    __shared__ uint32_t sumWave[4], maxWave[4];
// ... 229 lines not shown
        const uint32_t at = blockIdx.x * 256 + threadIdx.x;
        active = at < total;
        if (active) mine = W.sortedIdx[at];
        for (int i = threadIdx.x; i < 3 * (RT_GRID_DIV + 1); i += 256) planes[i] = S.boxMin[i];
        __syncthreads();
    } else {
        const uint32_t group = min(mode.groupRays, (uint32_t)RT_WF_GROUP_RAYS);
        __shared__ uint32_t pieceWave[4], pieceAt[2];
        uint32_t sl = 0, row = 0, count = 0;
        {
            static_assert(2 * RT_WF_SHARDS == 512, "two queue slices per thread");
            const uint32_t s0 = threadIdx.x, s1 = 256u + threadIdx.x;
            const uint32_t c0 = s0 < 2u * mode.slices ? slice_count(ctl, mode.slices, s0) : 0u, c1 = s1 < 2u * mode.slices ? slice_count(ctl, mode.slices, s1) : 0u;
            const uint32_t p0 = (c0 + group - 1u) / group, p1 = (c1 + group - 1u) / group;
            uint32_t i0 = p0, i1 = p1;
#pragma unroll
            for (int off = 1; off < 64; off <<= 1) {
                const uint32_t u0 = __shfl_up(i0, off, 64), u1 = __shfl_up(i1, off, 64);
                if ((int)lane >= off) { i0 += u0; i1 += u1; }
            }
            if (lane == 63) { pieceWave[wave] = i0; }
            __syncthreads();
            uint32_t before0 = 0, all0 = 0;
            for (uint32_t w = 0; w < 4; ++w) { if (w < wave) before0 += pieceWave[w]; all0 += pieceWave[w]; }
            __syncthreads();
            if (lane == 63) { pieceWave[wave] = i1; }
            __syncthreads();
            uint32_t before1 = all0, all1 = all0;
            for (uint32_t w = 0; w < 4; ++w) { if (w < wave) before1 += pieceWave[w]; all1 += pieceWave[w]; }
            const uint32_t first0 = before0 + i0 - p0, first1 = before1 + i1 - p1;
            if (blockIdx.x == 0 && threadIdx.x == 0 && all1 > gridDim.x) atomicOr(W.hostStatus + RT_WF_STATUS_ERROR, RT_WF_ERR_GRID);
            if (blockIdx.x >= all1) return;
            if (first0 <= blockIdx.x && blockIdx.x < first0 + p0) { pieceAt[0] = s0; pieceAt[1] = blockIdx.x - first0; }
            if (first1 <= blockIdx.x && blockIdx.x < first1 + p1) { pieceAt[0] = s1; pieceAt[1] = blockIdx.x - first1; }
            __syncthreads();
            sl = pieceAt[0]; row = pieceAt[1];
            count = slice_count(ctl, mode.slices, sl);
        }
        for (int i = threadIdx.x; i < 3 * (RT_GRID_DIV + 1); i += 256) planes[i] = S.boxMin[i];
        __syncthreads();
        const uint32_t rowsUsed = (count + group - 1u) / group;
        __shared__ uint32_t planWave[2];
        uint32_t n = 0;
        const uint32_t local = row + threadIdx.x * rowsUsed;
        const bool planner = threadIdx.x < group && local < count;
        if (planner) {
            const uint32_t q = slice_first(W, mode.slices, sl) + local;
            const uint4 *e = W.ent[par] + 4 * (size_t)q;
            const uint32_t excl = reinterpret_cast<const uint32_t *>(e)[3];
            const float tmin = __uint_as_float(reinterpret_cast<const uint32_t *>(e)[7]);
            const uint4 c2 = e[2], c3 = e[3];
            const V3 o = mk(__uint_as_float(c2.x), __uint_as_float(c2.y), __uint_as_float(c2.z)), d = mk(__uint_as_float(c3.x), __uint_as_float(c3.y), __uint_as_float(c3.z));
            const float tmax = __uint_as_float(c2.w);
            const EntryPlan plan = plan_ray(planes, o, d, tmin, tmax);
            n = segments_of(plan, d, tmax, mode.segLen);
            rayO[threadIdx.x] = pack4(o, tmin); rayD[threadIdx.x] = pack4(d, tmax);
            rayX[threadIdx.x] = make_uint4(excl, q, plan.start.cell, plan.endCell);
            rayT[threadIdx.x] = make_float4(plan.start.dx, plan.start.dy, plan.start.dz, plan.te);
        }
        if (wave < 2) {
            uint32_t sum = n;
#pragma unroll
            for (int off = 32; off >= 1; off >>= 1) sum += __shfl_xor(sum, off, 64);
            if (lane == 0) planWave[wave] = sum;
        }
        __syncthreads();
        const uint32_t all = planWave[0] + planWave[1];
        __syncthreads();
        if (wave < 2) {
            const uint32_t raysHere = min(group, (count - row + rowsUsed - 1u) / rowsUsed);
            if (all > 256u && n > 1u) n = max(1u, n * (256u - raysHere) / all);
            uint32_t incl = n;
#pragma unroll
            for (int off = 1; off < 64; off <<= 1) {
                const uint32_t up = __shfl_up(incl, off, 64);
                if ((int)lane >= off) incl += up;
            }
            if (lane == 63) planWave[wave] = incl;
            n = incl - n;
        }
        __syncthreads();
        if (wave < 2) {
            const uint32_t nextFirst = (uint32_t)__shfl_down((int)n, 1, 64);
            const uint32_t first = n + (wave == 1 ? planWave[0] : 0u), mineN = (lane == 63 ? planWave[wave] : nextFirst) - n;
            segFirst[threadIdx.x] = first;
            if (threadIdx.x == 127) segFirst[128] = planWave[0] + planWave[1];
            for (uint32_t k = 0; k < mineN; ++k) segOwner[first + k] = (uint8_t)threadIdx.x;
        }
        __syncthreads();
        segments = segFirst[128];
    }

    for (uint32_t pass = 0; pass < 1u; ++pass) {
    uint32_t q = 0, excluded = RT_NONE, cell = 0, endCell = 0xffffffffu, seg = 0;
    V3 o = mk(0, 0, 0), d = mk(1, 1, 1);
    float tmin = 0.f, tmax = 0.f, dx = 0.f, dy = 0.f, dz = 0.f;
    if (ORDERED) {
        if (active) {
            const uint4 *e = W.ent[par] + 4 * (size_t)mine;
            const uint4 c0 = e[0], c1 = e[1], c2 = e[2], c3 = e[3];
            q = c0.x; cell = c0.y & 0xffffffu; endCell = c0.z; excluded = c0.w;
            dx = __uint_as_float(c1.x); dy = __uint_as_float(c1.y); dz = __uint_as_float(c1.z); tmin = __uint_as_float(c1.w);
            o = mk(__uint_as_float(c2.x), __uint_as_float(c2.y), __uint_as_float(c2.z)); tmax = __uint_as_float(c2.w);
            d = mk(__uint_as_float(c3.x), __uint_as_float(c3.y), __uint_as_float(c3.z));
            seg = c3.w >> 24;
        }
    } else {
// ... 961 lines not shown
```

opencl_render_amd/csrc/rt_wf_logic_body.h:

```cpp
    __shared__ Shared sh;
    __shared__ float4 ltPosRadius[RT_WF_LIGHTS_LDS], ltDirSpread[RT_WF_LIGHTS_LDS], ltColHalf[RT_WF_LIGHTS_LDS];
    __shared__ int ltType[RT_WF_LIGHTS_LDS];
    __shared__ uint32_t waveHist[ORDERED ? 4 : 1][RT_WF_SORT_BINS], waveBase[ORDERED ? 4 : 1][RT_WF_SORT_BINS];
    __shared__ uint8_t cellLut[ORDERED ? 3 * 256 : 4];
    __shared__ uint8_t itemOwner[ORDERED ? 4 : 1][2 * 64 * (RT_WF_MAXSEG - 1)];
    __shared__ uint32_t itemWord[ORDERED ? 4 : 1][ORDERED ? 2 * 64 * (RT_WF_MAXSEG - 1) : 1];
    __shared__ float lutScale[3];
    static_assert(RT_WF_SORT_BINS == 64, "one class per lane");
    sh.unit255[threadIdx.x] = (float)threadIdx.x / 255.f;
    if (ORDERED) {
        float *pl = &sh.planes[0][0];
        for (int i = threadIdx.x; i < 3 * (RT_GRID_DIV + 1); i += 256) pl[i] = S.boxMin[i];
        waveHist[threadIdx.x >> 6][threadIdx.x & 63] = 0u;
        if (threadIdx.x < 3 * 256 / 4) reinterpret_cast<uint32_t *>(cellLut)[threadIdx.x] = reinterpret_cast<const uint32_t *>(S.cellLut)[threadIdx.x];
        if (threadIdx.x < 3) lutScale[threadIdx.x] = 256.f / (S.boxMin[threadIdx.x * (RT_GRID_DIV + 1) + RT_GRID_DIV] - S.boxMin[threadIdx.x * (RT_GRID_DIV + 1)]);
    }
    if (threadIdx.x < RT_WF_LIGHTS_LDS && threadIdx.x < S.lightCount) {
        const uint32_t k = threadIdx.x;
        ltType[k] = S.lightType[k];
        ltPosRadius[k] = make_float4(S.lightPos[4 * k], S.lightPos[4 * k + 1], S.lightPos[4 * k + 2], S.lightRadius[k]);
        ltDirSpread[k] = make_float4(S.lightDir[4 * k], S.lightDir[4 * k + 1], S.lightDir[4 * k + 2], S.lightSpread[k]);
        ltColHalf[k] = make_float4(S.lightCol[4 * k], S.lightCol[4 * k + 1], S.lightCol[4 * k + 2], S.lightHalfAtt[k]);
    }
    __syncthreads();
// ... 572 lines not shown
                    W.shFace[a] = pack4(face, front ? 1.f : 0.f);
                    if (attStored) W.shAtt[a] = pack4(atten, 0.f);
                    if (multiLight) {
                        W.rngL[a] = rngL;
                        if (shadedNow) W.shN[a] = pack4(n, 0.f);
                    }
                }
            }
        }
        uint32_t slot, slotLa;
        wave_append2(&ctlOut[RT_WF_CTL_COUNTS + outShard], emit, &ctlOut[RT_WF_CTL_COUNTS + RT_WF_SHARDS + outShard], emitLa, slot, slotLa);
        slot += outShard * sliceCapOut;
        slotLa += W.capacity + outShard * sliceCapOut;
        asm volatile("" : "+v"(a), "+v"(slot), "+v"(slotLa));
        if (slot != 0xfffffff0u) DG(8);
        const uint32_t copy = waveId % RT_WF_SORT_COPIES;
        if (!ORDERED) {
#pragma unroll 1
            for (int which = 0; which < 2; ++which) {
                const bool has = which ? emitLa : emit;
                if (!has) continue;
                const V3 o = which ? lo3 : ro, d = which ? ld3v : rd;
                const float tmin = which ? latmin : rtmin, tmax = which ? RT_INF : rtmax;
                const uint32_t excluded = which ? laexcl : rexcl, mine = which ? slotLa : slot;
                uint4 *e = W.ent[outq] + 4 * (size_t)mine;
                if (!which) W.pathOf[outq][mine] = make_uint2(a, emitLa ? slotLa : 0xffffffffu);
                W.hitKey[outq][mine] = ~0ull;
                reinterpret_cast<uint32_t *>(e)[3] = excluded;
                reinterpret_cast<uint32_t *>(e)[7] = __float_as_uint(tmin);
                e[2] = make_uint4(__float_as_uint(o.x), __float_as_uint(o.y), __float_as_uint(o.z), __float_as_uint(tmax));
                e[3] = make_uint4(__float_as_uint(d.x), __float_as_uint(d.y), __float_as_uint(d.z), 0u);
            }
        } else {
            auto visit_class = [](uint32_t v) -> uint32_t {
                if ((int)v < 1) v = 1;
                if (v > 767u) v = 767u;
                return (v < 128u) ? 63u - (v >> 2) : 31u - (v - 128u) / 20u;
            };
            EntryPlan planM, planL;
            planM.visits = planL.visits = 1; planM.endCell = planL.endCell = 0xffffffffu; planM.te = planL.te = RT_INF;
            planM.start.cell = planL.start.cell = 0; planM.start.dx = planM.start.dy = planM.start.dz = 0.f; planL.start.dx = planL.start.dy = planL.start.dz = 0.f;
            uint32_t nsegM = 0, nsegL = 0;
            const uint8_t *lut = next.segLen >= 4096u ? cellLut : nullptr;
#pragma unroll 1
            for (int which = 0; which < 2; ++which) {
                const bool has = which ? emitLa : emit;
                if (__ballot(has) == 0ull) continue;
                const V3 o = which ? lo3 : ro, d = which ? ld3v : rd;
                const float tmin = which ? latmin : rtmin, tmax = which ? RT_INF : rtmax;
                const bool sameStart = which && emit && lo3.x == ro.x && lo3.y == ro.y && lo3.z == ro.z && latmin == 0.f && rtmin == 0.f &&
                                       planes[0] <= o.x && o.x <= planes[RT_GRID_DIV] && planes[RT_GRID_DIV + 1] <= o.y && o.y <= planes[2 * RT_GRID_DIV + 1] &&
                                       planes[2 * (RT_GRID_DIV + 1)] <= o.z && o.z <= planes[3 * RT_GRID_DIV + 2];
                if (has) {
                    const EntryPlan plan = plan_ray(planes, o, d, tmin, tmax, sameStart, planM.start.cell, lut, lutScale);
                    const uint32_t n = segments_of(plan, d, tmax, next.segLen);
                    if (which) { planL = plan; nsegL = n; } else { planM = plan; nsegM = n; }
                }
            }
            const uint32_t extraM = nsegM > 1u ? nsegM - 1u : 0u, extraL = nsegL > 1u ? nsegL - 1u : 0u;
            uint32_t itemsM = 0, itemsL = 0, beforeM = 0, beforeL = 0;
            const bool cutting = __ballot((extraM | extraL) != 0u) != 0ull;
            if (cutting) {
                uint32_t inclM = extraM, inclL = extraL;
#pragma unroll
                for (int off = 1; off < 64; off <<= 1) {
                    const uint32_t upM = __shfl_up(inclM, off, 64), upL = __shfl_up(inclL, off, 64);
                    if ((int)lane >= off) { inclM += upM; inclL += upL; }
                }
                itemsM = (uint32_t)__shfl((int)inclM, 63, 64); itemsL = (uint32_t)__shfl((int)inclL, 63, 64);
                beforeM = inclM - extraM; beforeL = inclL - extraL;
            }
            const uint32_t items = itemsM + itemsL;
            uint32_t extraBase = 0;
            bool room = true;
            if (items != 0u) {
                if (lane == 0u) extraBase = atomicAdd(&ctlOut[RT_WF_CTL_EXTRA], items);
                extraBase = (uint32_t)__shfl((int)extraBase, 0, 64);
                if ((uint64_t)extraBase + items > (uint64_t)W.extraCap) {
                    room = false;
                    for (uint32_t i = extraBase + lane; i < W.extraCap; i += 64) {
                        W.ent[outq][4 * (size_t)(2u * W.capacity + i)].x = 0xffffffffu;
                        W.sortRank[2u * W.capacity + i] = 0xffffffffu;
                    }
                    if (nsegM > 1u) nsegM = 1u;
                    if (nsegL > 1u) nsegL = 1u;
                }
            }
            const uint32_t extraAt = 2u * W.capacity + extraBase;
            const float taM = fminf(planM.start.dx, fminf(planM.start.dy, planM.start.dz)), taL = fminf(planL.start.dx, fminf(planL.start.dy, planL.start.dz));
            const uint32_t perM = nsegM ? (planM.visits + nsegM - 1) / nsegM : 1u, perL = nsegL ? (planL.visits + nsegL - 1) / nsegL : 1u;
            uint32_t binM = 0, rankM = 0, binL = 0, rankL = 0;
            {
                float tau;
                if (emit) { binM = visit_class(nsegM > 1u && cut_at(taM, planM.te, 1u, nsegM, tau) ? perM : planM.visits); rankM = atomicAdd(&waveHist[wave][binM], 1u); }
                if (emitLa) { binL = visit_class(nsegL > 1u && cut_at(taL, planL.te, 1u, nsegL, tau) ? perL : planL.visits); rankL = atomicAdd(&waveHist[wave][binL], 1u); }
                if (cutting && room) {
#pragma unroll 1
                    for (int which = 0; which < 2; ++which) {
                        const uint32_t n = which ? nsegL : nsegM, per = which ? perL : perM, visits = which ? planL.visits : planM.visits;
                        const float ta = which ? taL : taM, te = which ? planL.te : planM.te;
                        const uint32_t at = which ? itemsM + beforeL : beforeM;
                        for (uint32_t k = 1; k < n; ++k) {
                            uint32_t word = 0xffffffffu;
                            if (cut_at(ta, te, k, n, tau)) {
                                const bool cutNext = k + 1u < n && cut_at(ta, te, k + 1u, n, tau);
                                const uint32_t bin = visit_class(cutNext ? per : visits - per * k);
                                word = atomicAdd(&waveHist[wave][bin], 1u) | (bin << 24);
// ... 114 lines not shown
```

opencl_render_amd/raytrace.py:

```python
from __future__ import annotations

import ctypes as C
import os
from typing import Optional, Sequence

import numpy as np

from .scene import GRID_DIV, Scene

_HERE = os.path.dirname(os.path.abspath(__file__))
LIB_PATH = os.environ.get("RT_HIP_LIB") or os.path.join(_HERE, "libraytrace_hip.so")
TILE = 128
PIPELINE_MEGAKERNEL, PIPELINE_WAVEFRONT = 0, 1
PASS_ALPHA, PASS_DEPTH, PASS_TRIANGLE, PASS_NORMAL, PASS_ALBEDO = 1, 2, 4, 8, 16


class Float3(C.Structure):
    _fields_ = [("s", C.c_float * 4)]


class UInt2(C.Structure):
    _fields_ = [("s", C.c_uint32 * 2)]


# ... 58 lines not shown
    _fields_ = [("width", C.c_uint32), ("height", C.c_uint32), ("raysPerTexel", C.c_uint32), ("radius", C.c_float), ("seed", C.c_uint32),
                ("dilate", C.c_uint32), ("firstTriangle", C.c_uint32), ("triangleCount", C.c_uint32), ("material", C.c_int32),
                ("matchMaterial", C.c_uint32)]


BAKE_DEFAULTS = dict(rays=16, radius=float("inf"), seed=0, dilate=2)
ALL_TRIANGLES = 0xFFFFFFFF


class Camera(C.Structure):
    _fields_ = [("eye", C.c_float * 4), ("eyeToTopLeft", C.c_float * 4), ("leftToRight", C.c_float * 4), ("topToBottom", C.c_float * 4),
                ("pixelSizeInv", C.c_float)]


class SampleWindow(C.Structure):
    _fields_ = [(n, C.c_uint32) for n in ("total", "first", "divisor", "accumulate", "advance")]

    def as_dict(self):
        return {n: int(getattr(self, n)) for n, _ in self._fields_}


class GeometryUpdate(C.Structure):
    _fields_ = [("vertexCount", C.c_uint32), ("vertex", C.c_void_p), ("triIndex", C.c_void_p), ("triNormal", C.c_void_p), ("arraysOnDevice", C.c_int32)]


class Stats(C.Structure):
    _fields_ = [(n, C.c_uint64) for n in ("primarySamples", "primaryCandidates", "gridRays", "gridCells", "gridCandidates", "shadedHits", "texelFetches")]

    def as_dict(self):
        return {n: int(getattr(self, n)) for n, _ in self._fields_}


DROPIN_SYMBOLS = [
    "RaytraceAll", "InitOpenCL", "ResetComputationType", "GetIsComputationTypeUpdated", "GetComputationTypeCount",
    "GetComputationTypeName", "GetProgress", "SetProgress", "GetStartTime", "GetEndTime", "ResetTime",
    "dot", "cross", "normalize", "vector", "bindf", "GetPointToLineSqLen", "RayIntersectsTriangle", "GetBoxAddress",
]
RESIDENT_SYMBOLS = [
    "rtHipCacheClear", "rtHipDeviceCount", "rtHipLastError", "rtHipSceneCreate", "rtHipSceneCreateLike", "rtHipSceneDestroy", "rtHipSceneBytes", "rtHipSceneGetCamera", "rtHipSceneSetCamera", "rtHipSceneSetGeometry", "rtHipRenderTiles", "rtHipFrameFinish",
    "rtHipSampleWindowCheck", "rtHipSceneSetSampleWindow", "rtHipSceneGetSampleWindow",
    "rtHipSetPipeline", "rtHipStageTiming", "rtHipStageTimes", "rtHipDebugCounters",
    "rtHipRenderTilesCounted", "rtHipTileBuffer", "rtHipTileBufferBytes", "rtHipDetile", "rtHipDetileStore", "rtHipDeviceAlloc", "rtHipDeviceFree", "rtHipDeviceCopy", "rtHipReadback", "rtHipSync",
    "rtHipScenePasses", "rtHipPassBuffer", "rtHipPassBufferBytes", "rtHipReadbackPasses",
    "rtHipSurfaceBuffer", "rtHipSurfaceBufferBytes", "rtHipReadbackSurfacePasses",
    "rtHipSceneIntersect", "rtHipSceneIntersectDevice",
    "rtHipDenoiseDefaults", "rtHipDenoiseScratchBytes", "rtHipDenoiseDevice", "rtHipDenoise", "rtHipSceneDenoise", "rtHipSceneDenoiseTimes",
    "rtHipAoDefaults", "rtHipSceneAmbientOcclusion", "rtHipSceneAmbientOcclusionDevice",
    "rtHipSceneMotionMark", "rtHipSceneMotionReferenceCamera", "rtHipSceneMotion", "rtHipSceneMotionDevice",
    "rtHipTemporalDefaults", "rtHipTemporalDevice", "rtHipTemporal", "rtHipSceneTemporal", "rtHipSceneTemporalReset", "rtHipSceneTemporalTimes",
    "rtHipVarianceDefaults", "rtHipTemporalMomentsDevice", "rtHipTemporalMoments", "rtHipVarianceScratchBytes", "rtHipDenoiseVarianceDevice",
    "rtHipDenoiseVariance", "rtHipSceneTemporalVariance",
    "rtHipBakeDefaults", "rtHipSceneBakeAmbientOcclusion", "rtHipSceneBakeAmbientOcclusionDevice",
    "rtHipKernelTime", "rtHipBuildCameraList", "rtHipBuildCameraListDevice", "rtHipBuildSceneGrid", "rtHipBuildSceneGridDevice", "rtHipFree",
    "rtHipDeviceKat", "rtHipTune", "rtHipTestCachePointers", "rtHipTestHashBytes", "rtHipScenePathClass", "rtHipTestPathClass", "rtHipTestRoundLog", "rtHipTestShadeLog", "rtHipTestBuildLog",
    "rtHipTestShadeKat", "rtHipTestSceneView", "rtHipTestSceneCameraList", "rtHipTestScenePointers", "rtHipTestSceneCameraLog", "rtHipTestSceneCameraTimes",
    "rtHipTestSceneGeometryLog", "rtHipTestSceneGeometryTimes",
    "rtHipSetCamera", "rtHipMeshCount", "rtHipMeshFill", "rtHipLightFill", "rtHipBakeMaterials", "rtHipPlanesToRgb8", "rtHipWriteBmp", "rtHipWritePpm", "rtHipWritePgm", "rtHipWritePfm", "rtHipWritePfmRgb",
    "rtHipObjRead", "rtHipObjFree", "rtHipImageRead", "rtHipProjectUv",
]

_lib = None


def lib() -> C.CDLL:
    global _lib
    if _lib is not None:
        return _lib
    if not os.path.exists(LIB_PATH):
        raise RuntimeError(f"{LIB_PATH} is missing: build it with `python -c 'import __graft_entry__ as g; g.build()'` "
                           "(there is no CPU fallback for the HIP path)")
    L = C.CDLL(LIB_PATH)
    vp, u32, u64, i32, f32 = C.c_void_p, C.c_uint32, C.c_uint64, C.c_int32, C.c_float
    L.RaytraceAll.restype = u32
    L.RaytraceAll.argtypes = [u32, UInt2, Float3, Float3, Float3, Float3, f32, vp, vp, vp, C.c_ssize_t, u32, u32, vp, u32, vp, vp, vp, vp,
                              i32, vp, vp, vp, u32, vp, vp, u32, vp, u32, vp, vp, vp, vp, vp, vp, vp, vp, vp]
    L.InitOpenCL.restype = None
    L.ResetComputationType.restype = None
    L.GetIsComputationTypeUpdated.restype = u32
    L.GetComputationTypeCount.restype = C.c_size_t
    L.GetComputationTypeName.restype = u32
    L.GetComputationTypeName.argtypes = [C.c_size_t, C.c_size_t, C.c_char_p]
    L.GetProgress.restype = f32
    L.SetProgress.argtypes = [f32]
    L.GetStartTime.restype = C.c_long
    L.GetEndTime.restype = C.c_long
    L.dot.restype = f32
    L.dot.argtypes = [Float3, Float3]
    L.cross.restype = Float3
    L.cross.argtypes = [Float3, Float3]
    L.normalize.restype = Float3
    L.normalize.argtypes = [Float3]
    L.vector.restype = Float3
    L.vector.argtypes = [Float3, Float3]
    L.bindf.restype = f32
    L.bindf.argtypes = [f32, f32, f32]
    L.GetPointToLineSqLen.restype = f32
    L.GetPointToLineSqLen.argtypes = [Float3, Float3, Float3]
    L.RayIntersectsTriangle.restype = u32
    L.RayIntersectsTriangle.argtypes = [Float3, Float3, f32, f32, Float3, Float3, Float3, C.POINTER(f32), C.POINTER(f32), C.POINTER(f32)]
    L.GetBoxAddress.restype = type("Int3", (C.Structure,), {"_fields_": [("s", C.c_int32 * 4)]})
    L.GetBoxAddress.argtypes = [i32, vp, Float3]

    L.rtHipCacheClear.restype = None
    L.rtHipDeviceCount.restype = C.c_int
    L.rtHipLastError.restype = C.c_char_p
    L.rtHipSceneCreate.restype = vp
    L.rtHipSceneCreate.argtypes = [C.c_int, C.POINTER(SceneDesc), vp, u32]
# ... 48 lines not shown
    L.rtHipReadbackSurfacePasses.argtypes = [vp, vp, vp]
    L.rtHipSceneIntersect.argtypes = [vp, vp, vp, u32, vp]
    L.rtHipSceneIntersectDevice.argtypes = [vp, vp, vp, u32, vp, vp]
    L.rtHipDenoiseDefaults.restype = None
    L.rtHipDenoiseDefaults.argtypes = [C.POINTER(DenoiseParams)]
    L.rtHipDenoiseScratchBytes.restype = u64
    L.rtHipDenoiseScratchBytes.argtypes = [u32, u32]
    L.rtHipDenoiseDevice.argtypes = [C.c_int, u32, u32, vp, vp, vp, vp, vp, u64, C.POINTER(DenoiseParams), vp]
    L.rtHipDenoise.argtypes = [C.c_int, u32, u32, vp, vp, vp, vp, C.POINTER(DenoiseParams)]
    L.rtHipSceneDenoise.argtypes = [vp, C.POINTER(DenoiseParams), vp, vp, vp, vp]
    L.rtHipSceneDenoiseTimes.argtypes = [vp, C.POINTER(C.c_float)]
    L.rtHipAoDefaults.restype = None
    L.rtHipAoDefaults.argtypes = [C.POINTER(AoParams)]
    L.rtHipSceneAmbientOcclusion.argtypes = [vp, C.POINTER(AoParams), vp]
    L.rtHipSceneAmbientOcclusionDevice.argtypes = [vp, C.POINTER(AoParams), vp, vp]
    L.rtHipSceneMotionMark.argtypes = [vp]
    L.rtHipSceneMotionReferenceCamera.argtypes = [vp, C.POINTER(Camera)]
    L.rtHipSceneMotion.argtypes = [vp, vp, vp, vp, vp]
    L.rtHipSceneMotionDevice.argtypes = [vp, vp, vp, vp, vp, vp]
    L.rtHipTemporalDefaults.restype = None
    L.rtHipTemporalDefaults.argtypes = [C.POINTER(TemporalParams)]
    L.rtHipTemporalDevice.argtypes = [C.c_int, u32, u32] + [vp] * 10 + [C.POINTER(TemporalParams), vp]
    L.rtHipTemporal.argtypes = [C.c_int, u32, u32] + [vp] * 10 + [C.POINTER(TemporalParams)]
    L.rtHipSceneTemporal.argtypes = [vp, C.POINTER(TemporalParams), C.POINTER(DenoiseParams), vp, vp, vp, vp, vp]
    L.rtHipSceneTemporalReset.argtypes = [vp]
    L.rtHipSceneTemporalTimes.argtypes = [vp, C.POINTER(C.c_float)]
    L.rtHipVarianceDefaults.restype = None
    L.rtHipVarianceDefaults.argtypes = [C.POINTER(VarianceParams)]
    L.rtHipTemporalMomentsDevice.argtypes = [C.c_int, u32, u32] + [vp] * 13 + [C.POINTER(TemporalParams), vp]
    L.rtHipTemporalMoments.argtypes = [C.c_int, u32, u32] + [vp] * 13 + [C.POINTER(TemporalParams)]
    L.rtHipVarianceScratchBytes.restype = C.c_uint64
    L.rtHipVarianceScratchBytes.argtypes = [u32, u32]
    L.rtHipDenoiseVarianceDevice.argtypes = [C.c_int, u32, u32] + [vp] * 8 + [C.c_uint64, C.POINTER(VarianceParams), vp]
    L.rtHipDenoiseVariance.argtypes = [C.c_int, u32, u32] + [vp] * 7 + [C.POINTER(VarianceParams)]
    L.rtHipSceneTemporalVariance.argtypes = [vp, C.POINTER(TemporalParams), C.POINTER(VarianceParams), vp, vp, vp, vp, vp, vp]
    L.rtHipBakeDefaults.restype = None
    L.rtHipBakeDefaults.argtypes = [C.POINTER(BakeParams)]
    L.rtHipSceneBakeAmbientOcclusion.argtypes = [vp, C.POINTER(BakeParams), vp, vp]
    L.rtHipSceneBakeAmbientOcclusionDevice.argtypes = [vp, C.POINTER(BakeParams), vp, vp, vp]
    L.rtHipKernelTime.argtypes = [vp, C.POINTER(C.c_double), C.POINTER(u64)]
    L.rtHipBuildCameraList.argtypes = [u32, u32, vp, vp, vp, vp, f32, u32, vp, vp, C.c_int,
                                       C.POINTER(vp), C.POINTER(vp), C.POINTER(vp), C.POINTER(u64)]
    L.rtHipBuildSceneGrid.argtypes = [u32, u32, vp, vp, C.c_int, vp, C.POINTER(vp), C.POINTER(vp), C.POINTER(u64)]
    L.rtHipBuildSceneGridDevice.argtypes = [C.c_int, u32, u32, vp, vp, vp, C.POINTER(vp), C.POINTER(vp), C.POINTER(u64), C.POINTER(C.c_double)]
    L.rtHipBuildCameraListDevice.argtypes = [C.c_int, u32, u32, vp, vp, vp, vp, f32, u32, u32, vp, vp,
                                             C.POINTER(vp), C.POINTER(vp), C.POINTER(vp), C.POINTER(u64), C.POINTER(C.c_double)]
    L.rtHipDeviceKat.argtypes = [C.c_int, C.c_int, u32, vp, u32, vp, u32, vp]
    L.rtHipTune.argtypes = [C.c_char_p, C.c_double]
    L.rtHipTestHashBytes.restype = u64
    L.rtHipTestHashBytes.argtypes = [vp, u64]
    L.rtHipScenePathClass.argtypes = [C.POINTER(SceneDesc)]
    L.rtHipTestPathClass.argtypes = [vp]
    L.rtHipTestRoundLog.argtypes = [vp, C.POINTER(u32), u32]
    L.rtHipTestShadeLog.argtypes = [vp, C.POINTER(u32), u32]
    L.rtHipTestBuildLog.argtypes = [C.POINTER(u64), u32]
    L.rtHipTestShadeKat.argtypes = [vp, C.c_int, u32, vp, vp]
    L.rtHipTestSceneView.argtypes = [vp, C.c_int, u64, u64, vp]
    L.rtHipFree.argtypes = [vp]
    L.rtHipFree.restype = None
    _lib = L
    return L


_ENV_KEYS = {
    "RT_HIP_STAGE_MB": "stage_mb", "RT_WF_EXTRA_FACTOR": "extra_factor", "RT_WF_STATE_MB": "state_mb", "RT_WF_GROUPS": "groups",
    "RT_WF_LOOKAHEAD": "lookahead", "RT_WF_FAST_QUOTIENT": "fast_quotient", "RT_WF_SPIN_LIMIT": "spin_limit",
    "RT_WF_APPEND_RAYS": "append_rays", "RT_WF_ORDERED_FIRST": "ordered_first", "RT_WF_SLICE_RAYS": "slice_rays", "RT_WF_SMALL_SLICES": "small_slices", "RT_WF_GROUP_RAYS": "group_rays",
    "RT_WF_BLOCKING": "blocking", "RT_WF_BATCH_PLAN": "batch_plan", "RT_WF_PLAN_ROUNDS": "plan_rounds", "RT_HIP_PIPELINE": "pipeline",
    "RT_HIP_TIMING": "timing", "RT_HIP_VIRTUAL_DEVICES": "virtual_devices", "RT_HIP_CACHE": "cache",
    "RT_WF_LOGIC_CLASS": "logic_class", "RT_WF_DEAD_SHADOW": "dead_shadow", "RT_WF_LOGIC_SPLIT": "logic_split", "RT_WF_PLAN_SHADE_SKIP": "plan_shade_skip",
    "RT_BUILD_KEY_CAP": "build_key_cap", "RT_BUILD_LIST_LIMIT": "build_list_limit", "RT_HIP_QUERY_RAYS": "query_rays",
}
_ENV_LISTS = (("RT_WF_SEG", "seg", 5), ("RT_WF_SEG_RAYS", "seg_rays", 4))


def tune(key: str, value: float) -> None:
    if lib().rtHipTune(key.encode(), float(value)) != 0:
        raise ValueError(last_error())


def apply_env_tuning() -> None:
    tune("reset", 0)
    for var, key in _ENV_KEYS.items():
        if var in os.environ:
            tune(key, float(os.environ[var]))
    for var, key, n in _ENV_LISTS:
        for i, v in enumerate([x for x in os.environ.get(var, "").split(",") if x][:n]):
            tune(f"{key}{i}", float(v))
    if os.environ.get("RT_WF_PLAN_GRID") == "tiny":
        tune("plan_grid_tiny", 1)


def last_error() -> str:
    return lib().rtHipLastError().decode("utf-8", "replace")


def _ptr(a):
    if a is None:
        return None
    if hasattr(a, "data_ptr"):
        return C.c_void_p(a.data_ptr())
    return a.ctypes.data_as(C.c_void_p)


def _f3(v) -> Float3:
    out = Float3()
    for i in range(3):
        out.s[i] = float(v[i])
    out.s[3] = 0.0
    return out


def _take(ptr: C.c_void_p, count: int, dtype) -> np.ndarray:
    n = max(int(count), 0)
    out = np.empty(n, dtype)
    if n:
        C.memmove(out.ctypes.data, ptr.value, n * out.itemsize)
    lib().rtHipFree(ptr)
    return out



def build_camera_list(sc: Scene, threads: int = 0) -> None:
# ... 305 lines not shown
    scratch = A.new(nbytes, np.uint8)
    if lib().rtHipDenoiseVarianceDevice(device, W, H, *ptrs, A.address(scratch), nbytes, C.byref(p), A.stream_arg()) != 0:
        raise RuntimeError("rtHipDenoiseVarianceDevice failed: " + last_error())
    A.done([v for _, v, _ in given] + list(res.values()) + [scratch])
    return res


def computation_type_names() -> list:
    L = lib()
    L.InitOpenCL()
    names = []
    buf = C.create_string_buffer(256)
    for i in range(L.GetComputationTypeCount()):
        if L.GetComputationTypeName(i, 255, buf):
            names.append(buf.value.decode())
    return names



def scene_desc(sc: Scene) -> SceneDesc:
    d = SceneDesc()
    d.width, d.height = sc.width, sc.height
    for i in range(4):
        d.eye[i] = float(sc.eye[i]); d.eyeToTopLeft[i] = float(sc.eye_to_top_left[i])
        d.leftToRight[i] = float(sc.left_to_right[i]); d.topToBottom[i] = float(sc.top_to_bottom[i])
    d.pixelSizeInv = sc.pixel_size_inv
    d.camStart, d.camEnd, d.camList = _ptr(sc.cam_start), _ptr(sc.cam_end), _ptr(sc.cam_list)
    d.camListSize = len(sc.cam_list)
    d.sampleCount = sc.sample_count
    d.vertexCount, d.vertex = sc.vertex_count, _ptr(sc.vertex)
    d.triangleCount = sc.triangle_count
    d.triIndex, d.triMaterial, d.triUv, d.triNormal = _ptr(sc.tri_index), _ptr(sc.tri_material), _ptr(sc.tri_uv), _ptr(sc.tri_normal)
    d.axesDiv = GRID_DIV
    d.boxMin, d.gridStart, d.gridList = _ptr(sc.box_min), _ptr(sc.grid_start), _ptr(sc.grid_list)
    d.materialCount, d.matSize, d.matStart = sc.material_count, _ptr(sc.mat_size), _ptr(sc.mat_start)
    d.texturesSize, d.textures = len(sc.textures), _ptr(sc.textures)
    d.lightCount, d.lightType = sc.light_count, _ptr(sc.light_type)
    d.lightPos, d.lightDir, d.lightCol = _ptr(sc.light_pos), _ptr(sc.light_dir), _ptr(sc.light_col)
    d.lightRadius, d.lightHalfAtt = _ptr(sc.light_radius), _ptr(sc.light_half_att)
    on_device = [bool(getattr(getattr(sc, k), "is_cuda", False)) for k in ("vertex", "tri_index", "cam_start", "grid_start", "textures", "light_type")]
    if any(on_device) and not all(on_device):
        raise ValueError("a scene's arrays must be all host arrays or all device tensors")
    d.arraysOnDevice = 1 if all(on_device) else 0
    return d


PATH_CLASS_GENERAL, PATH_CLASS_OPAQUE_DIFFUSE = 0, 1

SCENE_VIEWS = {
    "header": (0, np.uint32, 1), "cam_start": (1, np.uint32, 1), "cam_end": (2, np.uint32, 1), "tri_rec": (3, np.float32, 16),
    "tri_shade": (4, np.float32, 24), "grid_bits": (5, np.uint64, 1), "block_sparse": (6, np.uint32, 1), "pair_rec": (7, np.uint32, 16),
    "cell_lut": (8, np.uint8, 1),
}
SCENE_VIEW_HEADER = ("planes_tame", "tile_count", "tiles_x", "triangle_count", "pair_count")


def path_class(sc: Scene) -> int:
    d = SceneDesc()
    d.materialCount, d.matSize, d.matStart = sc.material_count, _ptr(sc.mat_size), _ptr(sc.mat_start)
    d.texturesSize, d.textures = len(sc.textures), _ptr(sc.textures)
    d.lightCount, d.lightType = sc.light_count, _ptr(sc.light_type)
    c = lib().rtHipScenePathClass(C.byref(d))
    if c < 0:
        raise ValueError(last_error())
    return c


def tile_count(width: int, height: int) -> int:
    return ((width + TILE - 1) // TILE) * ((height + TILE - 1) // TILE)


def tiles_of_rank(width: int, height: int, rank: int, world: int) -> np.ndarray:
    return np.arange(rank, tile_count(width, height), world, dtype=np.uint32)


def look_at_vectors(position, look_at, up, fov: float, width: int, height: int):
    from . import frontend
    return frontend.set_camera(position, look_at, up, fov, width, height)


def orbit_positions(position, look_at, count: int) -> list:
    p, c = np.asarray(position, np.float64)[:3], np.asarray(look_at, np.float64)[:3]
    dx, dz = p[0] - c[0], p[2] - c[2]
    out = []
    for i in range(count):
        a = 2.0 * np.pi * i / count
        out.append(np.array([c[0] + dx * np.cos(a) + dz * np.sin(a), p[1], c[2] - dx * np.sin(a) + dz * np.cos(a)], np.float64))
    return out


def orbit_path(path: str, index: int) -> str:
    import os
    root, ext = os.path.splitext(path)
    return f"{root}_{index:03d}{ext}"


def spin_vertices(points, centre, index: int, count: int) -> np.ndarray:
    src = np.asarray(points, np.float32)
    out = src.copy()
    if index % count == 0:
        return out
    c = np.asarray(centre, np.float64)
    a = 2.0 * np.pi * index / count
    dx, dz = src[:, 0].astype(np.float64) - c[0], src[:, 2].astype(np.float64) - c[2]
    out[:, 0] = c[0] + dx * np.cos(a) + dz * np.sin(a)
    out[:, 2] = c[2] - dx * np.sin(a) + dz * np.cos(a)
# ... 159 lines not shown
        sc.__dict__["_stale"] = {"grid", "camera"}
        self.scene = sc

    def set_vertices(self, vertex, tri_index=None, tri_normal=None) -> None:
        rc = self.try_set_vertices(vertex, tri_index, tri_normal)
        if rc != 0:
            raise RuntimeError(f"rtHipSceneSetGeometry failed ({rc}): {last_error()}")

    def geometry_log(self) -> dict:
        out = (C.c_uint64 * 6)()
        if lib().rtHipTestSceneGeometryLog(self.handle, C.byref(out), 6) != 6:
            raise RuntimeError("rtHipTestSceneGeometryLog failed: " + last_error())
        return dict(thread=int(out[0]), group=int(out[1]), attempts=int(out[2]), pairs=int(out[3]), entries=int(out[4]), allocated=int(out[5]))

    def geometry_times_ms(self) -> dict:
        out = (C.c_double * 4)()
        self._check(lib().rtHipTestSceneGeometryTimes(self.handle, C.byref(out)), "rtHipTestSceneGeometryTimes")
        return dict(records=out[0], grid=out[1], dense=out[2], camera=out[3])

    def camera_list(self, first: int = 0, count: Optional[int] = None) -> np.ndarray:
        total = lib().rtHipTestSceneCameraList(self.handle, 0, 0, None)
        if total < 0:
            raise RuntimeError("rtHipTestSceneCameraList failed: " + last_error())
        if count is None:
            count = max(total - first, 0)
        out = np.zeros(count, np.uint32)
        self._check(lib().rtHipTestSceneCameraList(self.handle, first, count, _ptr(out)), "rtHipTestSceneCameraList")
        return out

    def pointers(self) -> tuple:
        out = (C.c_void_p * 6)()
        self._check(lib().rtHipTestScenePointers(self.handle, C.byref(out)), "rtHipTestScenePointers")
        return tuple(int(v or 0) for v in out)

    def camera_log(self) -> dict:
        out = (C.c_uint64 * 3)()
        self._check(lib().rtHipTestSceneCameraLog(self.handle, C.byref(out)), "rtHipTestSceneCameraLog")
        return dict(thread=int(out[0]), group=int(out[1]), entries=int(out[2]))

    def camera_times_ms(self) -> dict:
        out = (C.c_double * 2)()
        self._check(lib().rtHipTestSceneCameraTimes(self.handle, C.byref(out)), "rtHipTestSceneCameraTimes")
        return dict(count=out[0], fill=out[1])

    def path_class(self) -> int:
        return lib().rtHipTestPathClass(self.handle)

    def round_rays(self, n: int = 8) -> list:
        rays = (C.c_uint32 * n)()
        if lib().rtHipTestRoundLog(self.handle, rays, n) < 0:
            raise RuntimeError("rtHipTestRoundLog failed")
        return [int(v) for v in rays]

    def shade_log(self, n: int = 8):
        listed = (C.c_uint32 * n)()
        rounds = lib().rtHipTestShadeLog(self.handle, listed, n)
        if rounds < 0:
            raise RuntimeError("rtHipTestShadeLog failed")
        return rounds, [int(v) for v in listed]

    def shade_kat(self, op: int, inp: np.ndarray) -> np.ndarray:
        inp = np.ascontiguousarray(inp)
        n = inp.shape[0]
        out = np.zeros((n, 64 if op == 0 else 96), np.uint8)
        self._check(lib().rtHipTestShadeKat(self.handle, op, n, _ptr(inp), _ptr(out)), "rtHipTestShadeKat")
        return out

    def scene_view(self, name: str, first: int = 0, count: Optional[int] = None) -> np.ndarray:
        what, dtype, words = SCENE_VIEWS[name]
        total = lib().rtHipTestSceneView(self.handle, what, 0, 0, None)
        if total < 0:
            raise RuntimeError("rtHipTestSceneView failed: " + last_error())
        if count is None:
            count = max(total - first, 0)
        out = np.zeros((count, words) if words > 1 else count, dtype)
        self._check(lib().rtHipTestSceneView(self.handle, what, first, count, _ptr(out)), "rtHipTestSceneView")
        return out

    def scene_header(self) -> dict:
        return dict(zip(SCENE_VIEW_HEADER, (int(v) for v in self.scene_view("header"))))

    def _check(self, rc, what):
        if rc != 0:
            raise RuntimeError(f"{what} failed: {last_error()}")

    def render(self, stream: int = 0):
        self._check(lib().rtHipRenderTiles(self.handle, stream or None), "rtHipRenderTiles")

    def finish(self) -> bool:
        redone = C.c_int(0)
        self._check(lib().rtHipFrameFinish(self.handle, C.byref(redone)), "rtHipFrameFinish")
        return bool(redone.value)

    def set_sample_window(self, total: Optional[int] = None, first: int = 0, divisor: Optional[int] = None, accumulate: bool = False,
                          advance: bool = False) -> None:
        S = int(self.scene.sample_count)
        w = SampleWindow(S if total is None else total, first, S if divisor is None else divisor, int(accumulate), int(advance))
        self._check(lib().rtHipSceneSetSampleWindow(self.handle, C.byref(w)), "rtHipSceneSetSampleWindow")

    def sample_window(self) -> dict:
        nxt, last = SampleWindow(), SampleWindow()
        self._check(lib().rtHipSceneGetSampleWindow(self.handle, C.byref(nxt), C.byref(last)), "rtHipSceneGetSampleWindow")
        return {"next": nxt.as_dict(), "last": last.as_dict()}

    def progressive(self, total: int, stream: int = 0):
        S = int(self.scene.sample_count)
        self.set_sample_window(total, 0, total, accumulate=True, advance=True)
        for done in range(S, int(total) + 1, S):
            self.render(stream)
            yield done, self.readback()

    def set_pipeline(self, pipeline: int):
        self._check(lib().rtHipSetPipeline(self.handle, pipeline), "rtHipSetPipeline")

    def stage_timing(self, enable: bool):
        self._check(lib().rtHipStageTiming(self.handle, 1 if enable else 0), "rtHipStageTiming")

    def stage_times_ms(self):
        ms, rounds = (C.c_double * 5)(), C.c_uint64()
        self._check(lib().rtHipStageTimes(self.handle, C.byref(ms), C.byref(rounds)), "rtHipStageTimes")
        return dict(primary=ms[0], logic=ms[1], trace=ms[2], accum=ms[3], sort=ms[4]), rounds.value

    def debug_counters(self, clear: bool = True):
        out = (C.c_uint64 * 8)()
        self._check(lib().rtHipDebugCounters(self.handle, C.byref(out), 1 if clear else 0), "rtHipDebugCounters")
        return [int(v) for v in out]

    def render_counted(self) -> dict:
        st = Stats()
        self._check(lib().rtHipRenderTilesCounted(self.handle, C.byref(st)), "rtHipRenderTilesCounted")
# ... 353 lines not shown
```

Baseline: 2715.

## Clip rays to tight occupied-geometry bounding planes before grid traversal

Adds a build-time pass that computes support distances of occupied grid blocks along a fixed set of candidate normals, picks up to a maximum number of clipping planes, and stores them after the grid plane table in the boxMin buffer. The ray entry planner then clips rays to this tighter convex hull, so rays end traversal earlier and visit fewer empty cells. It also adds a visit-count logging test hook and scene views. It costs extra build work, a host sync and a few plane tests per ray, and changes plan_ray/segments_of behaviour, which risks correctness at hull edges.

```diff
diff --git a/include/raytrace_hip.h b/include/raytrace_hip.h
--- a/include/raytrace_hip.h
+++ b/include/raytrace_hip.h
@@ -421,6 +421,9 @@
 
 int rtHipTestRoundLog(const rtHipScene *scene, cl_uint *rays, cl_uint n);
 
+enum { RT_ROUND_VISIT_ORDERED = 0, RT_ROUND_VISIT_ENTRIES, RT_ROUND_VISIT_ENDED, RT_ROUND_VISIT_RAYS, RT_ROUND_VISIT_FIELDS = 12 };
+int rtHipTestRoundVisits(const rtHipScene *scene, uint64_t *out, cl_uint rounds);
+
 int rtHipTestShadeLog(const rtHipScene *scene, cl_uint *listed, cl_uint n);
 
 enum { RT_BUILD_LOG_CAM_THREAD = 0, RT_BUILD_LOG_CAM_GROUP, RT_BUILD_LOG_CAM_ENTRIES, RT_BUILD_LOG_GRID_THREAD, RT_BUILD_LOG_GRID_GROUP,
@@ -429,7 +432,8 @@
 int rtHipTestBuildLog(uint64_t *out, cl_uint n);
 
 enum { RT_SCENE_VIEW_HEADER = 0, RT_SCENE_VIEW_CAM_START, RT_SCENE_VIEW_CAM_END, RT_SCENE_VIEW_TRI_REC, RT_SCENE_VIEW_TRI_SHADE,
-       RT_SCENE_VIEW_GRID_BITS, RT_SCENE_VIEW_BLOCK_SPARSE, RT_SCENE_VIEW_PAIR_REC, RT_SCENE_VIEW_CELL_LUT, RT_SCENE_VIEWS };
+       RT_SCENE_VIEW_GRID_BITS, RT_SCENE_VIEW_BLOCK_SPARSE, RT_SCENE_VIEW_PAIR_REC, RT_SCENE_VIEW_CELL_LUT, RT_SCENE_VIEWS,
+       RT_SCENE_VIEW_CLIP_PLANES = 16, RT_SCENE_VIEW_CLIP_APPLIED  };
 int rtHipTestSceneView(const rtHipScene *scene, int what, uint64_t firstElement, uint64_t count, void *out);
 
 int rtHipTestSceneCameraList(const rtHipScene *scene, uint64_t first, uint64_t count, cl_uint *out);
diff --git a/opencl_render_amd/csrc/rt_api.cpp b/opencl_render_amd/csrc/rt_api.cpp
--- a/opencl_render_amd/csrc/rt_api.cpp
+++ b/opencl_render_amd/csrc/rt_api.cpp
@@ -22,6 +22,8 @@
                                    hipStream_t stream);
 extern "C" hipError_t rtp_camera_ranges(uint32_t W, uint32_t H, uint32_t tilesX, const uint32_t *tileIds, uint32_t tileCount, const uint32_t *camStart,
                                         const uint32_t *camEnd, uint64_t camListSize, uint32_t *outStart, uint32_t *outEnd, uint32_t *err, hipStream_t stream);
+extern "C" hipError_t rtp_clip_support(const unsigned long long *words, const float *planeTable, const float *normals, uint32_t candidates, uint32_t *keys,
+                                       hipStream_t stream);
 extern "C" hipError_t rtp_dense_grid(const uint32_t *gridStart, const uint32_t *gridList, unsigned long long *words, uint32_t *sparse, uint32_t *pairOrder,
                                      uint32_t *pairCount, void *scratch, size_t *scratchBytes, hipStream_t stream);
 
@@ -203,6 +205,39 @@
     }
 }
 
+void clip_buffer_init(const float *planes, float *buffer)
+{
+    static const std::vector<float> normals = [] { std::vector<float> n(4 * RT_CLIP_CANDIDATES); (void)rt_clip_candidates(reinterpret_cast<float (*)[4]>(n.data())); return n; }();
+    memset(buffer, 0, sizeof(float) * RT_CLIP_FLOATS);
+    memcpy(buffer, planes, sizeof(float) * 3 * (RT_GRID_DIV + 1));
+    memcpy(buffer + RT_CLIP_NORMALS_AT, normals.data(), sizeof(float) * normals.size());
+}
+hipError_t clip_bound_issue(rtHipScene *sc, const unsigned long long *words, float *boxMin, hipStream_t st)
+{
+    uint32_t *keys = reinterpret_cast<uint32_t *>(boxMin + RT_CLIP_KEYS_AT);
+    const hipError_t e = rtp_clip_support(words, boxMin, boxMin + RT_CLIP_NORMALS_AT, RT_CLIP_CANDIDATES, keys, st);
+    if (e != hipSuccess) return e;
+    return hipMemcpyAsync(sc->clipKeys, keys, sizeof sc->clipKeys, hipMemcpyDeviceToHost, st);
+}
+hipError_t clip_bound_commit(const rtHipScene *sc, const float *planes, float *boxMin, hipStream_t st, uint32_t *count, float *tail)
+{
+    float normal[RT_CLIP_CANDIDATES][4], off[RT_CLIP_CANDIDATES];
+    (void)rt_clip_candidates(normal);
+    const float inflate = rt_clip_inflation(planes);
+    for (int c = 0; c < RT_CLIP_CANDIDATES; ++c) off[c] = sc->clipKeys[c] ? rt_clip_unkey(sc->clipKeys[c]) + inflate : std::nanf("");
+    int kept[RT_CLIP_MAX_PLANES];
+    const int n = rt_clip_choose(planes, normal, off, RT_CLIP_CANDIDATES, kept, nullptr);
+    memset(tail, 0, sizeof sc->clipTail);
+    for (int k = 0; k < n; ++k) {
+        float *row = tail + 4 + 4 * k;
+        row[0] = normal[kept[k]][0]; row[1] = normal[kept[k]][1]; row[2] = normal[kept[k]][2]; row[3] = off[kept[k]];
+    }
+    *count = (uint32_t)n;
+    const uint32_t applied = sc->tune.rayClip ? *count : 0u;
+    memcpy(tail, &applied, 4);
+    return hipMemcpyAsync(boxMin + RT_CLIP_AT, tail, sizeof sc->clipTail, hipMemcpyHostToDevice, st);
+}
+
 int build_grid(rtHipScene *sc, const rtHipSceneDesc *d)
 {
     sc->release_part(PART_GRID);
@@ -212,7 +247,9 @@
     std::vector<float> planes(3 * (RT_GRID_DIV + 1));
     for (int w = 0; w < 3; ++w)
         for (int i = 0; i <= RT_GRID_DIV; ++i) planes[w * (RT_GRID_DIV + 1) + i] = d->boxMin[i].s[w];
-    if (sc->upload(planes.data(), planes.size(), &D.boxMin, "boxMin")) return -1;
+    std::vector<float> planeBuffer(RT_CLIP_FLOATS);
+    clip_buffer_init(planes.data(), planeBuffer.data());
+    if (sc->upload(planeBuffer.data(), planeBuffer.size(), &D.boxMin, "boxMin")) return -1;
     std::vector<uint8_t> lut(3 * 256);
     grid_tables(planes.data(), lut.data(), &D.planesTame);
     if (sc->upload(lut.data(), lut.size(), &D.cellLut, "cellLut")) return -1;
@@ -240,6 +277,7 @@
     HIP_OK(scratch.get((void **)&pairOrder, (size_t)listSize * 4)); HIP_OK(scratch.get((void **)&pairCount, (size_t)listSize * 4));
     HIP_OK(scratch.get(&tmp, tmpBytes));
     HIP_OK(rtp_dense_grid(D.gridStart, D.gridList, words, sparse, pairOrder, pairCount, tmp, &tmpBytes, sc->stream));
+    HIP_OK(clip_bound_issue(sc, words, const_cast<float *>(D.boxMin), sc->stream));
     float *pairRec = nullptr;
     if (sc->alloc<float>((uint64_t)listSize * 16, &pairRec)) return -1;
     HIP_OK(rtk_launch_gather_pairs((uint32_t)listSize, pairOrder, pairCount, D.triRec, pairRec, sc->stream));
@@ -247,6 +285,12 @@
     sc->gridListSize = listSize;
     D.cellCount = 0;
     HIP_OK(hipStreamSynchronize(sc->stream));
+    uint32_t clipCount = 0;
+    float clipTail[4 + 4 * RT_CLIP_MAX_PLANES];
+    HIP_OK(clip_bound_commit(sc, planes.data(), const_cast<float *>(D.boxMin), sc->stream, &clipCount, clipTail));
+    HIP_OK(hipStreamSynchronize(sc->stream));
+    sc->clipCount = clipCount;
+    memcpy(sc->clipTail, clipTail, sizeof sc->clipTail);
     return 0;
 }
 
@@ -455,7 +499,7 @@
     }
 }
 
-constexpr uint64_t GEO_PLANE_BYTES = 3 * (RT_GRID_DIV + 1) * 4, GEO_LUT_BYTES = 3 * 256, GEO_START_BYTES = ((uint64_t)RT_GRID_DIV * RT_GRID_DIV * RT_GRID_DIV + 1) * 4,
+constexpr uint64_t GEO_PLANE_BYTES = RT_CLIP_FLOATS * 4 , GEO_LUT_BYTES = 3 * 256, GEO_START_BYTES = ((uint64_t)RT_GRID_DIV * RT_GRID_DIV * RT_GRID_DIV + 1) * 4,
                    GEO_BITS_BYTES = (uint64_t)(RT_GRID_DIV / 4) * (RT_GRID_DIV / 4) * (RT_GRID_DIV / 4) * 8,
                    GEO_SPARSE_BYTES = (uint64_t)3 * ((63u << 16 | 63u << 8 | 63u) + 1u) * 4;
 
@@ -493,6 +537,11 @@
     if (part == PART_GRID) {
         D.planesTame = S.planesTame; D.cellCount = S.cellCount; dst->gridListSize = src->gridListSize;
         RT_MOVE(boxMin); RT_MOVE(cellLut); RT_MOVE(gridStart); RT_MOVE(gridList); RT_MOVE(gridBits); RT_MOVE(gridBlockSparse); RT_MOVE(pairRec);
+        dst->clipCount = src->clipCount;
+        memcpy(dst->clipTail, src->clipTail, sizeof dst->clipTail);
+        const uint32_t applied = dst->tune.rayClip ? dst->clipCount : 0u;
+        memcpy(dst->clipTail, &applied, 4);
+        HIP_OK(hipMemcpyAsync(const_cast<float *>(D.boxMin) + RT_CLIP_AT, dst->clipTail, 4, hipMemcpyHostToDevice, dst->stream));
     }
     if (part == PART_MATERIALS) {
         D.materialCount = S.materialCount; D.texelCount = S.texelCount; RT_MOVE(matSize); RT_MOVE(matStart); RT_MOVE(textures); RT_MOVE(matRec);
@@ -598,6 +647,71 @@
     return m;
 }
 
+int log_round_visits(rtHipScene *sc, rtHipScene::Group &G, uint32_t r, const RtRoundMode &mode, hipStream_t on)
+{
+    const RtWavefront &W = G.wf;
+    HIP_OK(hipStreamSynchronize(on));
+    std::vector<uint32_t> ctl(RT_WF_CTL_WORDS);
+    std::vector<float> planes(3 * (RT_GRID_DIV + 1));
+    HIP_OK(hipMemcpy(ctl.data(), W.ctl + (size_t)(r % 3) * RT_WF_CTL_WORDS, sizeof(uint32_t) * RT_WF_CTL_WORDS, hipMemcpyDeviceToHost));
+    HIP_OK(hipMemcpy(planes.data(), G.dev.boxMin, sizeof(float) * planes.size(), hipMemcpyDeviceToHost));
+    const uint32_t cap = W.capacity, sliceCap = cap / mode.slices;
+    const uint32_t extra = mode.ordered ? std::min(ctl[RT_WF_CTL_EXTRA], W.extraCap) : 0u;
+    std::vector<uint4> ent((size_t)4 * (2 * (size_t)cap + extra));
+    std::vector<unsigned long long> key(2 * (size_t)cap);
+    std::vector<uint2> pathOf(cap);
+    HIP_OK(hipMemcpy(ent.data(), W.ent[r & 1u], sizeof(uint4) * ent.size(), hipMemcpyDeviceToHost));
+    HIP_OK(hipMemcpy(key.data(), W.hitKey[r & 1u], sizeof(unsigned long long) * key.size(), hipMemcpyDeviceToHost));
+    HIP_OK(hipMemcpy(pathOf.data(), W.pathOf[r & 1u], sizeof(uint2) * pathOf.size(), hipMemcpyDeviceToHost));
+    auto cell_of = [&](const float p[3]) {
+        uint32_t c[3] = { 0, 0, 0 };
+        for (int w = 0; w < 3; ++w)
+            for (int div = RT_GRID_DIV / 2; div >= 1; div /= 2)
+                if (planes[(size_t)w * (RT_GRID_DIV + 1) + c[w] + div] < p[w]) c[w] += div;
+        return c[0] | c[1] << 8 | c[2] << 16;
+    };
+    auto visits_of = [&](const uint4 *e) -> uint64_t {
+        const uint32_t start = e[0].y & 0xffffffu;
+        uint32_t last = e[0].z;
+        if (last == 0xffffffffu) {
+            float o[3], d[3], te = HUGE_VALF;
+            memcpy(o, &e[2], 12); memcpy(d, &e[3], 12);
+            for (int w = 0; w < 3; ++w)
+                if (d[w] != 0.f) { const float t = (planes[(size_t)w * (RT_GRID_DIV + 1) + (0.f <= d[w] ? RT_GRID_DIV : 0)] - o[w]) / d[w]; if (t < te) te = t; }
+            if (!(te < HUGE_VALF)) return 1;
+            const float to[3] = { o[0] + te * d[0], o[1] + te * d[1], o[2] + te * d[2] };
+            last = cell_of(to);
+        }
+        uint64_t v = 1;
+        for (int w = 0; w < 3; ++w) v += (uint64_t)std::abs((int)((last >> 8 * w) & 255u) - (int)((start >> 8 * w) & 255u));
+        return v;
+    };
+    uint64_t *out = sc->visitLog[r].data();
+    out[RT_ROUND_VISIT_ORDERED] = mode.ordered;
+    auto kind_of = [&](uint32_t q) { return q >= cap ? 2u : (pathOf[q].y != 0xffffffffu ? 0u : 1u); };
+    for (uint32_t look = 0; look < 2; ++look)
+        for (uint32_t s = 0; s < mode.slices; ++s) {
+            const uint32_t n = std::min(ctl[RT_WF_CTL_COUNTS + look * RT_WF_SHARDS + s], sliceCap), base = look * cap + s * sliceCap;
+            for (uint32_t q = base; q < base + n; ++q) {
+                uint64_t *f = out + RT_ROUND_VISIT_RAYS + 3 * kind_of(q);
+                f[0] += 1;
+                f[1] += key[q] != ~0ull;
+                if (!mode.ordered) continue;
+                f[2] += visits_of(&ent[(size_t)4 * q]);
+                out[RT_ROUND_VISIT_ENTRIES] += 1;
+                out[RT_ROUND_VISIT_ENDED] += ent[(size_t)4 * q].z != 0xffffffffu;
+            }
+        }
+    for (uint32_t i = 0; i < extra; ++i) {
+        const uint4 *e = &ent[(size_t)4 * (2 * (size_t)cap + i)];
+        if (e[0].x >= 2 * cap) continue;
+        out[RT_ROUND_VISIT_RAYS + 3 * kind_of(e[0].x) + 2] += visits_of(e);
+        out[RT_ROUND_VISIT_ENTRIES] += 1;
+        out[RT_ROUND_VISIT_ENDED] += e[0].z != 0xffffffffu;
+    }
+    return 0;
+}
+
 int render_wavefront(rtHipScene *sc, hipStream_t st, bool forceDiscovery)
 {
     const Tuning &T = sc->tune;
@@ -619,6 +733,7 @@
         if (er != hipSuccess) return er;
         return hipEventRecord(e.b, on);
     };
+    if (T.visitLog) sc->visitLog.assign(RT_WF_ROUND_LOG, {});
     const bool serial = sc->stageTiming || sc->groups.size() == 1;
     auto streamOf = [&](size_t g) { return (serial || g == 0) ? st : sc->groups[g].stream; };
     if (!serial) {
@@ -662,6 +777,7 @@
         if (r > 0) {
             if (mode.ordered) HIP_OK(stage(4, on, [&] { return rtw_launch_scatter(&G.wf, r, G.queueBlocks, &mode, on); }));
             HIP_OK(stage(2, on, [&] { return rtw_launch_trace(&G.dev, &G.wf, r, trace_blocks(G, r, mode), &mode, on); }));
+            if (T.visitLog && r < RT_WF_ROUND_LOG && log_round_visits(sc, G, r, mode, on) != 0) return -1;
         }
         const RtRoundMode next = round_mode(G, r + 1);
         if (r > 0 && T.logicSplit && G.wf.lookAhead && G.dev.pathClass == RT_PATH_CLASS_OPAQUE_DIFFUSE) {
@@ -1801,7 +1917,9 @@
     for (int w = 0; w < 3; ++w)
         for (int i = 0; i <= RT_GRID_DIV; ++i) planes[w * (RT_GRID_DIV + 1) + i] = bm[4 * i + w];
     grid_tables(planes, lut, &tame);
-    GEO_HIP(hipMemcpyAsync(N.boxMin, planes, sizeof planes, hipMemcpyHostToDevice, st));
+    float planeBuffer[RT_CLIP_FLOATS];
+    clip_buffer_init(planes, planeBuffer);
+    GEO_HIP(hipMemcpyAsync(N.boxMin, planeBuffer, sizeof planeBuffer, hipMemcpyHostToDevice, st));
     GEO_HIP(hipMemcpyAsync(N.cellLut, lut, sizeof lut, hipMemcpyHostToDevice, st));
     GEO_HIP(hipEventRecord(G.ev[2], st));
 
@@ -1812,6 +1930,7 @@
     GEO_HIP(hipMemsetAsync(N.sparse, 0, GEO_SPARSE_BYTES, st));
     GEO_HIP(rtp_dense_grid(N.gridStart, N.gridList, N.gridBits, N.sparse, G.pairOrder, G.pairInfo, G.denseTmp, &denseBytes, st));
     GEO_HIP(rtk_launch_gather_pairs((uint32_t)pairs, G.pairOrder, G.pairInfo, N.triRec, N.pairRec, st));
+    GEO_HIP(clip_bound_issue(sc, N.gridBits, N.boxMin, st));
     GEO_HIP(hipEventRecord(G.ev[3], st));
 
     rtHipCamera cam;
@@ -1824,12 +1943,18 @@
     GEO_HIP(hipStreamSynchronize(st));
     float ms[4] = {};
     for (int i = 0; i < 4; ++i) GEO_HIP(hipEventElapsedTime(&ms[i], G.ev[i], G.ev[i + 1]));
+    uint32_t clipCount = 0;
+    float clipTail[4 + 4 * RT_CLIP_MAX_PLANES];
+    GEO_HIP(clip_bound_commit(sc, planes, N.boxMin, st, &clipCount, clipTail));
+    GEO_HIP(hipStreamSynchronize(st));
 #undef GEO_HIP
 #undef GEO_MEM
 
     RtDevScene &D = sc->dev;
     D.triRec = N.triRec; D.triShade = N.triShade;
     D.boxMin = N.boxMin; D.cellLut = N.cellLut; D.planesTame = tame;
+    sc->clipCount = clipCount;
+    memcpy(sc->clipTail, clipTail, sizeof sc->clipTail);
     D.gridStart = N.gridStart; D.gridList = N.gridList; D.gridBits = N.gridBits; D.gridBlockSparse = N.sparse; D.pairRec = N.pairRec;
     sc->gridListSize = pairs;
     G.live = target;
@@ -2041,9 +2166,9 @@
         { "seg0", &T.segLen[0] }, { "seg1", &T.segLen[1] }, { "seg2", &T.segLen[2] }, { "seg3", &T.segLen[3] }, { "seg4", &T.segLen[4] },
         { "seg_rays0", &T.segRays[0] }, { "seg_rays1", &T.segRays[1] }, { "seg_rays2", &T.segRays[2] }, { "seg_rays3", &T.segRays[3] },
         { "fast_quotient", &T.fastQuotient }, { "spin_limit", &T.spinLimit }, { "append_rays", &T.appendRays }, { "ordered_first", &T.orderedFirst }, { "slice_rays", &T.sliceRays },
-        { "small_slices", &T.smallSlices }, { "group_rays", &T.groupRays }, { "blocking", &T.blocking }, { "plan_rounds", &T.planRounds }, { "plan_grid_tiny", &T.planGridTiny }, { "plan_shade_skip", &T.planShadeSkip },
+        { "small_slices", &T.smallSlices }, { "group_rays", &T.groupRays }, { "blocking", &T.blocking }, { "plan_rounds", &T.planRounds }, { "plan_grid_tiny", &T.planGridTiny }, { "plan_shade_skip", &T.planShadeSkip }, { "visit_log", &T.visitLog },
         { "pipeline", &T.pipeline }, { "timing", &T.timing }, { "virtual_devices", &T.virtualDevices }, { "cache", &T.cache }, { "batch_plan", &T.batchPlan },
-        { "logic_class", &T.logicClass }, { "dead_shadow", &T.deadShadow }, { "logic_split", &T.logicSplit }, { "query_rays", &T.queryRays, nullptr, 1u << 26 },
+        { "logic_class", &T.logicClass }, { "dead_shadow", &T.deadShadow }, { "ray_clip", &T.rayClip }, { "logic_split", &T.logicSplit }, { "query_rays", &T.queryRays, nullptr, 1u << 26 },
         { "ao_samples", &T.aoSamples, nullptr, 1u << 22 }, { "bake_texels", &T.bakeTexels, nullptr, 1u << 24 },
         { "state_mb", nullptr, &T.stateMb, HUGE_VAL }, { "build_key_cap", nullptr, &T.buildKeyCap, 1e18 }, { "build_list_limit", nullptr, &T.buildListLimit },
     };
@@ -2102,6 +2227,15 @@
         rays[r] = (uint32_t)std::min<uint64_t>(sum, 0xffffffffu);
     }
     return (int)scene->roundsLast;
+}
+
+int rtHipTestRoundVisits(const rtHipScene *scene, uint64_t *out, uint32_t rounds)
+{
+    if (!scene || (rounds && !out)) return fail("rtHipTestRoundVisits: null argument");
+    if (!scene->tune.visitLog) return fail("rtHipTestRoundVisits: the scene was built without the test hook visit_log");
+    for (uint32_t r = 0; r < rounds; ++r)
+        for (uint32_t f = 0; f < RT_ROUND_VISIT_FIELDS; ++f) out[(size_t)RT_ROUND_VISIT_FIELDS * r + f] = r < scene->visitLog.size() ? scene->visitLog[r][f] : 0;
+    return (int)std::min<uint64_t>(scene->roundsLast, 0x7fffffffu);
 }
 
 int rtHipTestShadeLog(const rtHipScene *scene, uint32_t *listed, uint32_t n)
@@ -2134,6 +2268,8 @@
     case RT_SCENE_VIEW_BLOCK_SPARSE: v = { D.gridBlockSparse, (uint64_t)3 * ((63u << 16 | 63u << 8 | 63u) + 1u), 4, false }; break;
     case RT_SCENE_VIEW_PAIR_REC: v = { D.pairRec, scene->gridListSize, 64, false }; break;
     case RT_SCENE_VIEW_CELL_LUT: v = { D.cellLut, 3 * 256, 1, false }; break;
+    case RT_SCENE_VIEW_CLIP_PLANES: v = { D.boxMin ? D.boxMin + RT_CLIP_AT + 4 : nullptr, scene->clipCount, 16, false }; break;
+    case RT_SCENE_VIEW_CLIP_APPLIED: v = { D.boxMin ? D.boxMin + RT_CLIP_AT : nullptr, 1, 4, false }; break;
     default: return fail("rtHipTestSceneView: unknown array %d", what);
     }
     if (v.elements > 0x7fffffffull) return fail("rtHipTestSceneView: array %d has %llu elements", what, (unsigned long long)v.elements);
diff --git a/opencl_render_amd/csrc/rt_host.h b/opencl_render_amd/csrc/rt_host.h
--- a/opencl_render_amd/csrc/rt_host.h
+++ b/opencl_render_amd/csrc/rt_host.h
@@ -1,6 +1,7 @@
 #pragma once
 #include "raytrace_hip.h"
 #include "rt_device.h"
+#include "rt_ray_clip.h"
 #include "rt_camera_move.h"
 #include "rt_geometry_move.h"
 #include "rt_owned.h"
@@ -8,6 +9,7 @@
 #include <hip/hip_runtime_api.h>
 
 #include <algorithm>
+#include <array>
 #include <atomic>
 #include <cstring>
 #include <mutex>
@@ -48,6 +50,7 @@
     uint32_t planRounds = 0;
     uint32_t planGridTiny = 0;
     uint32_t planShadeSkip = 0;
+    uint32_t visitLog = 0;
     uint32_t pipeline = RT_HIP_PIPELINE_WAVEFRONT;
     uint32_t timing = 0;
     uint32_t virtualDevices = 0;
@@ -55,6 +58,7 @@
     uint32_t batchPlan = 1;
     uint32_t logicClass = 1;
     uint32_t deadShadow = 1;
+    uint32_t rayClip = 1;
     uint32_t logicSplit = 1;
     uint64_t buildKeyCap = 0;
     uint64_t buildListLimit = 0xffffffffull;
@@ -181,6 +185,9 @@
     uint64_t gridListSize = 0;
     uint32_t gridListSizeHint = 0;
     bool haveGridListSize = false;
+    uint32_t clipCount = 0;
+    float clipTail[4 + 4 * RT_CLIP_MAX_PLANES] = {};
+    uint32_t clipKeys[RT_CLIP_CANDIDATES] = {};
     bool wfMultiLight = false;
     bool classMaterials = false, classLights = false;
     uint64_t bytes = 0;
@@ -225,6 +232,7 @@
     size_t stageEventsUsed = 0;
     bool stageTiming = false;
     uint64_t roundsLast = 0;
+    std::vector<std::array<uint64_t, RT_ROUND_VISIT_FIELDS>> visitLog;
     uint32_t passMask = 0;
     rthost::Dev<uint32_t> passBuf;
     rthost::Dev<float> surfBuf;
diff --git a/opencl_render_amd/csrc/rt_ray_clip.h b/opencl_render_amd/csrc/rt_ray_clip.h
--- /dev/null
+++ b/opencl_render_amd/csrc/rt_ray_clip.h
@@ -0,0 +1,169 @@
+#ifndef RT_RAY_CLIP_H
+#define RT_RAY_CLIP_H
+
+#include <stddef.h>
+#include <stdint.h>
+
+#if defined(__HIPCC__) || defined(__CUDACC__)
+#define RT_CLIP_HD __host__ __device__ __forceinline__
+#else
+#define RT_CLIP_HD inline
+#endif
+
+#define RT_CLIP_MAX_PLANES 8
+#define RT_CLIP_CANDIDATES 290
+#define RT_CLIP_LATTICE 32
+
+#define RT_CLIP_AT 772
+#define RT_CLIP_PLANES_AT 776
+#define RT_CLIP_KEYS_AT (RT_CLIP_PLANES_AT + 4 * RT_CLIP_MAX_PLANES)
+#define RT_CLIP_NORMALS_AT (RT_CLIP_KEYS_AT + (RT_CLIP_CANDIDATES + 3) / 4 * 4)
+#define RT_CLIP_FLOATS (RT_CLIP_NORMALS_AT + 4 * RT_CLIP_CANDIDATES)
+
+#define RT_CLIP_SLACK_REL 2e-5f
+#define RT_CLIP_SLACK_ABS 2e-5f
+
+inline int rt_clip_candidates(float (*out)[4])
+{
+    auto gcd = [](int a, int b) { a = a < 0 ? -a : a; b = b < 0 ? -b : b; while (b) { const int t = a % b; a = b; b = t; } return a; };
+    int n = 0;
+    for (int z = -3; z <= 3; ++z)
+        for (int y = -3; y <= 3; ++y)
+            for (int x = -3; x <= 3; ++x) {
+                if (gcd(gcd(x, y), z) != 1) continue;
+                const double len = __builtin_sqrt((double)(x * x + y * y + z * z));
+                if (out) { out[n][0] = (float)(x / len); out[n][1] = (float)(y / len); out[n][2] = (float)(z / len); out[n][3] = 0.f; }
+                ++n;
+            }
+    return n;
+}
+
+RT_CLIP_HD uint32_t rt_clip_key(float f)
+{
+    union { float f; uint32_t u; } v; v.f = f;
+    return (v.u & 0x80000000u) ? ~v.u : (v.u | 0x80000000u);
+}
+RT_CLIP_HD float rt_clip_unkey(uint32_t k)
+{
+    union { float f; uint32_t u; } v; v.u = (k & 0x80000000u) ? (k & 0x7fffffffu) : ~k;
+    return v.f;
+}
+
+RT_CLIP_HD float rt_clip_support(float nx, float ny, float nz, float lox, float loy, float loz, float hix, float hiy, float hiz)
+{
+    return nx * (0.f <= nx ? hix : lox) + ny * (0.f <= ny ? hiy : loy) + nz * (0.f <= nz ? hiz : loz);
+}
+
+inline float rt_clip_inflation(const float *planes, int div = 256)
+{
+    float diag2 = 0.f, big = 0.f;
+    for (int w = 0; w < 3; ++w) {
+        const float lo = planes[w * (div + 1)], hi = planes[w * (div + 1) + div];
+        diag2 += (hi - lo) * (hi - lo);
+        const float a = lo < 0.f ? -lo : lo, b = hi < 0.f ? -hi : hi;
+        if (a > big) big = a;
+        if (b > big) big = b;
+    }
+    return 3e-4f * __builtin_sqrtf(diag2) + 2e-5f * big;
+}
+
+inline int rt_clip_choose(const float *planes, const float (*normal)[4], const float *off, int candidates, int *kept, int *cut, int div = 256)
+{
+    constexpr int L = RT_CLIP_LATTICE, WORDS = L * L;
+    static_assert(L == 32, "one word per lattice row");
+    float centre[3][L];
+    for (int w = 0; w < 3; ++w)
+        for (int i = 0; i < L; ++i) { const int c = (2 * i + 1) * div / (2 * L); centre[w][i] = 0.5f * (planes[w * (div + 1) + c] + planes[w * (div + 1) + c + 1]); }
+    uint32_t *mask = new uint32_t[(size_t)candidates * WORDS];
+    for (int c = 0; c < candidates; ++c) {
+        uint32_t *m = mask + (size_t)c * WORDS;
+        float ax[L];
+        for (int i = 0; i < L; ++i) ax[i] = normal[c][0] * centre[0][i];
+        const bool usable = off[c] == off[c] && off[c] - off[c] == 0.f;
+        for (int k = 0; k < L; ++k)
+            for (int j = 0; j < L; ++j) {
+                const float rest = off[c] - (normal[c][1] * centre[1][j] + normal[c][2] * centre[2][k]);
+                uint32_t word = 0;
+                if (usable) {
+                    int count = 0;
+                    if (normal[c][0] > 0.f) { int lo = 0, hi = L; while (lo < hi) { const int mid = (lo + hi) / 2; if (ax[mid] > rest) hi = mid; else lo = mid + 1; } count = L - lo; }
+                    else if (normal[c][0] < 0.f) { int lo = 0, hi = L; while (lo < hi) { const int mid = (lo + hi) / 2; if (ax[mid] > rest) lo = mid + 1; else hi = mid; } count = lo; }
+                    else count = ax[0] > rest ? L : 0;
+                    if (count) word = normal[c][0] > 0.f ? ~0u << (L - count) : ~0u >> (L - count);
+                }
+                m[k * L + j] = word;
+            }
+    }
+    uint32_t gone[WORDS] = {};
+    int *bound = new int[candidates];
+    for (int c = 0; c < candidates; ++c) bound[c] = L * L * L;
+    int n = 0, total = 0;
+    while (n < RT_CLIP_MAX_PLANES) {
+        int best = -1, bestGain = 0;
+        for (int c = 0; c < candidates; ++c) {
+            if (bound[c] <= bestGain) continue;
+            const uint32_t *m = mask + (size_t)c * WORDS;
+            int gain = 0;
+            for (int i = 0; i < WORDS; ++i) gain += __builtin_popcount(m[i] & ~gone[i]);
+            bound[c] = gain;
+            if (gain > bestGain) { bestGain = gain; best = c; }
+        }
+        if (best < 0) break;
+        const uint32_t *m = mask + (size_t)best * WORDS;
+        for (int i = 0; i < WORDS; ++i) gone[i] |= m[i];
+        kept[n++] = best;
+        total += bestGain;
+    }
+    delete[] mask;
+    delete[] bound;
+    if (total * 20 < L * L * L) n = 0, total = 0;
+    if (cut) *cut = total;
+    return n;
+}
+
+RT_CLIP_HD bool rt_clip_plain(bool farEnd, float dx, float dy, float dz, float te, float hx, float hy, float hz)
+{
+    const float inf = __builtin_inff();
+    const float ta = __builtin_fminf(hx, __builtin_fminf(hy, hz));
+    return !farEnd && dx != 0.f && dy != 0.f && dz != 0.f && te < inf && -inf < ta && ta < te && hx == hx && hy == hy && hz == hz && hx < inf &&
+           hy < inf && hz < inf;
+}
+
+#if defined(__HIP_DEVICE_COMPILE__)
+#define RT_CLIP_RCP(x) __builtin_amdgcn_rcpf(x)
+#else
+#define RT_CLIP_RCP(x) (1.f / (x))
+#endif
+
+RT_CLIP_HD float rt_clip_plane(float nx, float ny, float nz, float off, float ox, float oy, float oz, float dx, float dy, float dz, float tmin, float te)
+{
+    const float nd = nx * dx + ny * dy + nz * dz;
+    if (!(nd > 0.f)) return te;
+    const float ax = nx * ox, ay = ny * oy, az = nz * oz;
+    float num = off - (ax + ay + az);
+    num += RT_CLIP_SLACK_ABS * (__builtin_fabsf(off) + __builtin_fabsf(ax) + __builtin_fabsf(ay) + __builtin_fabsf(az));
+    float t = num * RT_CLIP_RCP(nd);
+    t += RT_CLIP_SLACK_REL * __builtin_fabsf(t);
+    return (tmin < t && t < te) ? t : te;
+}
+
+template <class P> RT_CLIP_HD float rt_clip_te(P clip, uint32_t count, float ox, float oy, float oz, float dx, float dy, float dz, float tmin, float te)
+{
+    for (uint32_t k = 0; k < count; ++k) {
+        const int at = (RT_CLIP_PLANES_AT - RT_CLIP_AT) + 4 * (int)k;
+        te = rt_clip_plane(clip[at], clip[at + 1], clip[at + 2], clip[at + 3], ox, oy, oz, dx, dy, dz, tmin, te);
+    }
+    return te;
+}
+
+template <class P> RT_CLIP_HD bool rt_clip_ray(P clip, uint32_t count, bool farEnd, bool startInside, float ox, float oy, float oz, float dx, float dy, float dz,
+                                               float tmin, float hx, float hy, float hz, float &te)
+{
+    if (count == 0u || !startInside || !rt_clip_plain(farEnd, dx, dy, dz, te, hx, hy, hz)) return false;
+    const float lowered = rt_clip_te(clip, count, ox, oy, oz, dx, dy, dz, tmin, te);
+    if (!(lowered < te)) return false;
+    te = lowered;
+    return true;
+}
+
+#endif
diff --git a/opencl_render_amd/csrc/rt_scene_prep.hip b/opencl_render_amd/csrc/rt_scene_prep.hip
--- a/opencl_render_amd/csrc/rt_scene_prep.hip
+++ b/opencl_render_amd/csrc/rt_scene_prep.hip
@@ -2,6 +2,7 @@
 #include <hipcub/hipcub.hpp>
 
 #include "rt_device.h"
+#include "rt_ray_clip.h"
 
 namespace {
 
@@ -97,6 +98,43 @@
     }
 }
 
+#define RTP_CLIP_NORMALS 16
+__global__ __launch_bounds__(256) void rtp_clip_support_kernel(const unsigned long long *__restrict__ words, const float *__restrict__ planeTable,
+                                                               const float4 *__restrict__ normals, uint32_t candidates, uint32_t *__restrict__ keys)
+{
+    __shared__ float pl[3 * (RT_GRID_DIV + 1)];
+    for (int i = threadIdx.x; i < 3 * (RT_GRID_DIV + 1); i += 256) pl[i] = planeTable[i];
+    __syncthreads();
+    const uint32_t b = blockIdx.x * 256 + threadIdx.x;
+    const uint32_t bx = b & 63u, by = (b >> 6) & 63u, bz = b >> 12;
+    const uint32_t first = blockIdx.y * RTP_CLIP_NORMALS;
+    unsigned long long w = words[b];
+    if (__ballot(w != 0ull) == 0ull) return;
+    float4 n[RTP_CLIP_NORMALS];
+    float best[RTP_CLIP_NORMALS];
+#pragma unroll
+    for (int j = 0; j < RTP_CLIP_NORMALS; ++j) {
+        n[j] = normals[min(first + j, candidates - 1u)];
+        best[j] = -__builtin_inff();
+    }
+    while (w) {
+        const int bit = __ffsll((long long)w) - 1;
+        w &= w - 1;
+        const uint32_t cx = bx * 4 + (bit & 3), cy = by * 4 + ((bit >> 2) & 3), cz = bz * 4 + (bit >> 4);
+        const float lox = pl[cx], hix = pl[cx + 1], loy = pl[(RT_GRID_DIV + 1) + cy], hiy = pl[(RT_GRID_DIV + 1) + cy + 1];
+        const float loz = pl[2 * (RT_GRID_DIV + 1) + cz], hiz = pl[2 * (RT_GRID_DIV + 1) + cz + 1];
+#pragma unroll
+        for (int j = 0; j < RTP_CLIP_NORMALS; ++j) best[j] = fmaxf(best[j], rt_clip_support(n[j].x, n[j].y, n[j].z, lox, loy, loz, hix, hiy, hiz));
+    }
+#pragma unroll
+    for (int j = 0; j < RTP_CLIP_NORMALS; ++j) {
+        float m = best[j];
+#pragma unroll
+        for (int off = 32; off >= 1; off >>= 1) m = fmaxf(m, __shfl_xor(m, off, 64));
+        if ((threadIdx.x & 63) == 0 && first + j < candidates && m > -__builtin_inff()) atomicMax(&keys[first + j], rt_clip_key(m));
+    }
+}
+
 }
 
 extern "C" hipError_t rtp_validate(uint32_t T, uint32_t V, uint32_t M, const void *triIndex, const int *triMaterial, uint64_t camListSize,
@@ -139,3 +177,14 @@
                        pairCount);
     return hipGetLastError();
 }
+
+extern "C" hipError_t rtp_clip_support(const unsigned long long *words, const float *planeTable, const float *normals, uint32_t candidates, uint32_t *keys,
+                                       hipStream_t stream)
+{
+    if (!candidates) return hipSuccess;
+    hipError_t e = hipMemsetAsync(keys, 0, sizeof(uint32_t) * candidates, stream);
+    if (e != hipSuccess) return e;
+    hipLaunchKernelGGL(rtp_clip_support_kernel, dim3(BLOCKS / 256, (candidates + RTP_CLIP_NORMALS - 1) / RTP_CLIP_NORMALS), dim3(256), 0, stream, words,
+                       planeTable, (const float4 *)normals, candidates, keys);
+    return hipGetLastError();
+}
diff --git a/opencl_render_amd/csrc/rt_wavefront.hip b/opencl_render_amd/csrc/rt_wavefront.hip
--- a/opencl_render_amd/csrc/rt_wavefront.hip
+++ b/opencl_render_amd/csrc/rt_wavefront.hip
@@ -1,4 +1,5 @@
 #include "rt_devfuncs.h"
+#include "rt_ray_clip.h"
 
 namespace {
 
@@ -310,13 +311,15 @@
 
 struct EntryPlan { DdaState start; uint32_t endCell, visits; float te; };
 
+typedef const __attribute__((address_space(4))) float *ClipPlanes;
 __device__ __forceinline__ EntryPlan plan_ray(const float *planes, V3 o, V3 d, float tmin, float tmax, bool haveStart = false, uint32_t startCell = 0u,
-                                              const uint8_t *lut = nullptr, const float *lutScale = nullptr)
+                                              const uint8_t *lut = nullptr, const float *lutScale = nullptr, const float *clip = nullptr)
 {
     EntryPlan p;
     const V3 lo = mk(planes[0], planes[RT_GRID_DIV + 1], planes[2 * (RT_GRID_DIV + 1)]);
     const V3 hi = mk(planes[RT_GRID_DIV], planes[2 * RT_GRID_DIV + 1], planes[3 * RT_GRID_DIV + 2]);
     V3 from = along(o, tmin, d);
+    const bool startInside = lo.x <= from.x && from.x <= hi.x && lo.y <= from.y && from.y <= hi.y && lo.z <= from.z && from.z <= hi.z;
     bind_in_cube(from, d, lo, hi);
     p.start.cell = startCell;
     if (!haveStart) p.start.cell = cell_of(planes, from);
@@ -331,27 +334,31 @@
         if (d.z != 0.f) { const float t = (((0.f <= d.z) ? hi.z : lo.z) - o.z) / d.z; if (t < p.te) p.te = t; }
         to = (p.te < RT_INF) ? along(o, p.te, d) : from;
     }
+    const int cx = (int)(p.start.cell & 255u), cy = (int)((p.start.cell >> 8) & 255u), cz = (int)(p.start.cell >> 16);
+    p.start.dx = (planes[cx + ((0 <= d.x) ? 1 : 0)] - o.x) / d.x;
+    p.start.dy = (planes[(RT_GRID_DIV + 1) + cy + ((0 <= d.y) ? 1 : 0)] - o.y) / d.y;
+    p.start.dz = (planes[2 * (RT_GRID_DIV + 1) + cz + ((0 <= d.z) ? 1 : 0)] - o.z) / d.z;
+    bool clipped = false;
+    if (clip) {
+        const ClipPlanes cp = (ClipPlanes)(uintptr_t)clip;
+        const uint32_t count = __float_as_uint(cp[0]);
+        clipped = rt_clip_ray(cp, count, tmax < RT_INF, startInside, o.x, o.y, o.z, d.x, d.y, d.z, tmin, p.start.dx, p.start.dy, p.start.dz, p.te);
+        if (clipped) to = along(o, p.te, d);
+    }
     uint32_t last;
-    if (lut && !(tmax < RT_INF)) {
+    if (lut && !(tmax < RT_INF) && !clipped) {
         const float fx = (to.x - lo.x) * lutScale[0], fy = (to.y - lo.y) * lutScale[1], fz = (to.z - lo.z) * lutScale[2];
         const int ix = min(255, max(0, (int)fx)), iy = min(255, max(0, (int)fy)), iz = min(255, max(0, (int)fz));
         last = (uint32_t)lut[ix] | ((uint32_t)lut[256 + iy] << 8) | ((uint32_t)lut[512 + iz] << 16);
     } else last = cell_of(planes, to);
-    p.endCell = (tmax < RT_INF) ? last : 0xffffffffu;
-    const int cx = (int)(p.start.cell & 255u), cy = (int)((p.start.cell >> 8) & 255u), cz = (int)(p.start.cell >> 16);
-    p.start.dx = (planes[cx + ((0 <= d.x) ? 1 : 0)] - o.x) / d.x;
-    p.start.dy = (planes[(RT_GRID_DIV + 1) + cy + ((0 <= d.y) ? 1 : 0)] - o.y) / d.y;
-    p.start.dz = (planes[2 * (RT_GRID_DIV + 1) + cz + ((0 <= d.z) ? 1 : 0)] - o.z) / d.z;
+    p.endCell = (tmax < RT_INF || clipped) ? last : 0xffffffffu;
     p.visits = (uint32_t)(abs((int)(last & 255u) - cx) + abs((int)((last >> 8) & 255u) - cy) + abs((int)(last >> 16) - cz)) + 1u;
     return p;
 }
 
 __device__ __forceinline__ uint32_t segments_of(const EntryPlan &p, V3 d, float tmax, uint32_t segLen)
 {
-    const float ta = fminf(p.start.dx, fminf(p.start.dy, p.start.dz));
-    const bool plain = !(tmax < RT_INF) && d.x != 0.f && d.y != 0.f && d.z != 0.f && p.te < RT_INF && -RT_INF < ta && ta < p.te &&
-                       p.start.dx == p.start.dx && p.start.dy == p.start.dy && p.start.dz == p.start.dz && p.start.dx < RT_INF &&
-                       p.start.dy < RT_INF && p.start.dz < RT_INF;
+    const bool plain = rt_clip_plain(tmax < RT_INF, d.x, d.y, d.z, p.te, p.start.dx, p.start.dy, p.start.dz);
     if (!plain || p.visits <= segLen + segLen / 4) return 1u;
     const uint32_t n = (p.visits + segLen - 1) / segLen;
     return n > RT_WF_MAXSEG ? (uint32_t)RT_WF_MAXSEG : n;
@@ -687,7 +694,7 @@
             const uint4 c2 = e[2], c3 = e[3];
             const V3 o = mk(__uint_as_float(c2.x), __uint_as_float(c2.y), __uint_as_float(c2.z)), d = mk(__uint_as_float(c3.x), __uint_as_float(c3.y), __uint_as_float(c3.z));
             const float tmax = __uint_as_float(c2.w);
-            const EntryPlan plan = plan_ray(planes, o, d, tmin, tmax);
+            const EntryPlan plan = plan_ray(planes, o, d, tmin, tmax, false, 0u, nullptr, nullptr, S.boxMin + RT_CLIP_AT);
             n = segments_of(plan, d, tmax, mode.segLen);
             rayO[threadIdx.x] = pack4(o, tmin); rayD[threadIdx.x] = pack4(d, tmax);
             rayX[threadIdx.x] = make_uint4(excl, q, plan.start.cell, plan.endCell);
diff --git a/opencl_render_amd/csrc/rt_wf_logic_body.h b/opencl_render_amd/csrc/rt_wf_logic_body.h
--- a/opencl_render_amd/csrc/rt_wf_logic_body.h
+++ b/opencl_render_amd/csrc/rt_wf_logic_body.h
@@ -648,7 +648,7 @@
                                        planes[0] <= o.x && o.x <= planes[RT_GRID_DIV] && planes[RT_GRID_DIV + 1] <= o.y && o.y <= planes[2 * RT_GRID_DIV + 1] &&
                                        planes[2 * (RT_GRID_DIV + 1)] <= o.z && o.z <= planes[3 * RT_GRID_DIV + 2];
                 if (has) {
-                    const EntryPlan plan = plan_ray(planes, o, d, tmin, tmax, sameStart, planM.start.cell, lut, lutScale);
+                    const EntryPlan plan = plan_ray(planes, o, d, tmin, tmax, sameStart, planM.start.cell, lut, lutScale, S.boxMin + RT_CLIP_AT);
                     const uint32_t n = segments_of(plan, d, tmax, next.segLen);
                     if (which) { planL = plan; nsegL = n; } else { planM = plan; nsegM = n; }
                 }
diff --git a/opencl_render_amd/raytrace.py b/opencl_render_amd/raytrace.py
--- a/opencl_render_amd/raytrace.py
+++ b/opencl_render_amd/raytrace.py
@@ -134,7 +134,7 @@
     "rtHipDenoiseVariance", "rtHipSceneTemporalVariance",
     "rtHipBakeDefaults", "rtHipSceneBakeAmbientOcclusion", "rtHipSceneBakeAmbientOcclusionDevice",
     "rtHipKernelTime", "rtHipBuildCameraList", "rtHipBuildCameraListDevice", "rtHipBuildSceneGrid", "rtHipBuildSceneGridDevice", "rtHipFree",
-    "rtHipDeviceKat", "rtHipTune", "rtHipTestCachePointers", "rtHipTestHashBytes", "rtHipScenePathClass", "rtHipTestPathClass", "rtHipTestRoundLog", "rtHipTestShadeLog", "rtHipTestBuildLog",
+    "rtHipDeviceKat", "rtHipTune", "rtHipTestCachePointers", "rtHipTestHashBytes", "rtHipScenePathClass", "rtHipTestPathClass", "rtHipTestRoundLog", "rtHipTestRoundVisits", "rtHipTestShadeLog", "rtHipTestBuildLog",
     "rtHipTestShadeKat", "rtHipTestSceneView", "rtHipTestSceneCameraList", "rtHipTestScenePointers", "rtHipTestSceneCameraLog", "rtHipTestSceneCameraTimes",
     "rtHipTestSceneGeometryLog", "rtHipTestSceneGeometryTimes",
     "rtHipSetCamera", "rtHipMeshCount", "rtHipMeshFill", "rtHipLightFill", "rtHipBakeMaterials", "rtHipPlanesToRgb8", "rtHipWriteBmp", "rtHipWritePpm", "rtHipWritePgm", "rtHipWritePfm", "rtHipWritePfmRgb",
@@ -289,6 +289,7 @@
     L.rtHipScenePathClass.argtypes = [C.POINTER(SceneDesc)]
     L.rtHipTestPathClass.argtypes = [vp]
     L.rtHipTestRoundLog.argtypes = [vp, C.POINTER(u32), u32]
+    L.rtHipTestRoundVisits.argtypes = [vp, C.POINTER(C.c_uint64), u32]
     L.rtHipTestShadeLog.argtypes = [vp, C.POINTER(u32), u32]
     L.rtHipTestBuildLog.argtypes = [C.POINTER(u64), u32]
     L.rtHipTestShadeKat.argtypes = [vp, C.c_int, u32, vp, vp]
@@ -305,7 +306,7 @@
     "RT_WF_APPEND_RAYS": "append_rays", "RT_WF_ORDERED_FIRST": "ordered_first", "RT_WF_SLICE_RAYS": "slice_rays", "RT_WF_SMALL_SLICES": "small_slices", "RT_WF_GROUP_RAYS": "group_rays",
     "RT_WF_BLOCKING": "blocking", "RT_WF_BATCH_PLAN": "batch_plan", "RT_WF_PLAN_ROUNDS": "plan_rounds", "RT_HIP_PIPELINE": "pipeline",
     "RT_HIP_TIMING": "timing", "RT_HIP_VIRTUAL_DEVICES": "virtual_devices", "RT_HIP_CACHE": "cache",
-    "RT_WF_LOGIC_CLASS": "logic_class", "RT_WF_DEAD_SHADOW": "dead_shadow", "RT_WF_LOGIC_SPLIT": "logic_split", "RT_WF_PLAN_SHADE_SKIP": "plan_shade_skip",
+    "RT_WF_LOGIC_CLASS": "logic_class", "RT_WF_DEAD_SHADOW": "dead_shadow", "RT_WF_RAY_CLIP": "ray_clip", "RT_WF_LOGIC_SPLIT": "logic_split", "RT_WF_PLAN_SHADE_SKIP": "plan_shade_skip", "RT_WF_VISIT_LOG": "visit_log",
     "RT_BUILD_KEY_CAP": "build_key_cap", "RT_BUILD_LIST_LIMIT": "build_list_limit", "RT_HIP_QUERY_RAYS": "query_rays",
 }
 _ENV_LISTS = (("RT_WF_SEG", "seg", 5), ("RT_WF_SEG_RAYS", "seg_rays", 4))
@@ -717,6 +718,9 @@
     "tri_shade": (4, np.float32, 24), "grid_bits": (5, np.uint64, 1), "block_sparse": (6, np.uint32, 1), "pair_rec": (7, np.uint32, 16),
     "cell_lut": (8, np.uint8, 1),
 }
+SCENE_VIEW_CLIP_PLANES = 16
+SCENE_VIEW_CLIP_APPLIED = 17
+ROUND_VISIT_FIELDS = 12
 SCENE_VIEW_HEADER = ("planes_tame", "tile_count", "tiles_x", "triangle_count", "pair_count")
 
 
@@ -982,6 +986,20 @@
             raise RuntimeError("rtHipTestRoundLog failed")
         return [int(v) for v in rays]
 
+    def round_visits(self, n: int = 8) -> list:
+        out = (C.c_uint64 * (ROUND_VISIT_FIELDS * n))()
+        if lib().rtHipTestRoundVisits(self.handle, out, n) < 0:
+            raise RuntimeError("rtHipTestRoundVisits failed: " + last_error())
+        rounds = []
+        for r in range(n):
+            f = [int(v) for v in out[ROUND_VISIT_FIELDS * r:ROUND_VISIT_FIELDS * (r + 1)]]
+            row = dict(ordered=f[0], entries=f[1], ended=f[2])
+            for k, kind in enumerate(("shadow", "main", "bounce")):
+                row[kind] = dict(rays=f[3 + 3 * k], hits=f[4 + 3 * k], visits=f[5 + 3 * k])
+            row["visits"] = sum(row[kind]["visits"] for kind in ("shadow", "main", "bounce"))
+            rounds.append(row)
+        return rounds
+
     def shade_log(self, n: int = 8):
         listed = (C.c_uint32 * n)()
         rounds = lib().rtHipTestShadeLog(self.handle, listed, n)
@@ -1006,6 +1024,20 @@
         out = np.zeros((count, words) if words > 1 else count, dtype)
         self._check(lib().rtHipTestSceneView(self.handle, what, first, count, _ptr(out)), "rtHipTestSceneView")
         return out
+
+    def clip_planes(self) -> np.ndarray:
+        total = lib().rtHipTestSceneView(self.handle, SCENE_VIEW_CLIP_PLANES, 0, 0, None)
+        if total < 0:
+            raise RuntimeError("rtHipTestSceneView failed: " + last_error())
+        out = np.zeros((total, 4), np.float32)
+        if total:
+            self._check(lib().rtHipTestSceneView(self.handle, SCENE_VIEW_CLIP_PLANES, 0, total, _ptr(out)), "rtHipTestSceneView")
+        return out
+
+    def clip_applied(self) -> int:
+        out = np.zeros(1, np.uint32)
+        self._check(lib().rtHipTestSceneView(self.handle, SCENE_VIEW_CLIP_APPLIED, 0, 1, _ptr(out)), "rtHipTestSceneView")
+        return int(out[0])
 
     def scene_header(self) -> dict:
         return dict(zip(SCENE_VIEW_HEADER, (int(v) for v in self.scene_view("header"))))
```

Result: faster. 2820, median of 6 (+3.9%).
